# fujii-team/Henbun

Measured on AMD Instinct MI355X. Metric: elbo_samples_per_sec, higher is better.
Workload: dtype f32; 1 GPU; cfg2 SVGP ELBO step: 1-D UnitRBF, N=1e6, M=512 inducing, minibatch 8192 per GPU, diag Normal q(u), diagonal residual, Adam lr 1e-3; global_batch=8192, per_gpu_batch=8192, parallelism=dp1, N=1000000, M=512, dp_exchange=none, dp_ranks=1, contraction=native, tri_pack=False

## Files before the change

henbun_amd/csrc/elementwise.hip:

```cpp
#include "common.cuh"
#include "rng_pairs.cuh"
#include "side_jobs.cuh"
#include <string.h>
#include "../../include/henbun_hip.h"

struct EwArgs {
  int ndim;
  int nin, nout;
  int op;
  long n;
  int shape[HB_MAX_DIMS];
  long istride[4][HB_MAX_DIMS];
  const void* in[4];
  void* out[3];
  double p[4];
};

#include "ew_apply.cuh"

template <typename T>
__global__ void __launch_bounds__(256) ew_kernel(EwArgs A) {
  const long stride = (long)gridDim.x * blockDim.x;
  for (long i = (long)blockIdx.x * blockDim.x + threadIdx.x; i < A.n; i += stride) {
    long off[4] = {0, 0, 0, 0};
// ... 618 lines not shown
                                                                     const long* __restrict__ perm, long n, long nsrc,
                                                                     int* __restrict__ err) {
  gather_draw_body<T>(g, state, nlanes, lo, range, idx_out, perm, n, nsrc, err, G, (long)blockIdx.x);
}
template <typename T>
static int gather_rows_multi_draw(int narr, const T* const* srcs, const long* rows, T* const* dsts, long nsrc,
                                  uint64_t* state, long nlanes, long lo, long hi, long* idx_out, const long* perm,
                                  long n, int* err, hipStream_t stream, bool defer = false) {
  HB_REQUIRE(narr >= 1 && narr <= HB_GATHER_MAX, "hb_gather_rows_multi_draw: %d arrays (max %d)", narr, HB_GATHER_MAX);
  HB_REQUIRE(n >= 0 && nsrc >= 0 && srcs && rows && dsts && state && idx_out, "hb_gather_rows_multi_draw: bad arguments");
  HB_REQUIRE(n <= nlanes, "hb_gather_rows_multi_draw: n=%ld exceeds the %ld RNG lanes (draw with hb_rng_randint instead)", n,
             nlanes);
  HB_REQUIRE(hi > lo, "hb_gather_rows_multi_draw: empty range [%ld,%ld)", lo, hi);
  GatherMultiArgs<T> g;
  g.narr = narr;
  g.start[0] = 0;
  long wmax = 1;
  for (int a = 0; a < HB_GATHER_MAX; ++a) {
    g.src[a] = a < narr ? srcs[a] : nullptr;
    g.dst[a] = a < narr ? dsts[a] : nullptr;
    g.row[a] = a < narr ? rows[a] : 1;
    if (a < narr) HB_REQUIRE(rows[a] >= 1 && srcs[a] && dsts[a], "hb_gather_rows_multi_draw: bad array %d", a);
    if (a < narr && rows[a] > wmax) wmax = rows[a];
    g.start[a + 1] = g.start[a] + (a < narr ? n * rows[a] : 0);
  }
  if (n == 0) return 0;
  const uint64_t range = (uint64_t)(hi - lo);
  constexpr long VEC = 16 / (long)sizeof(T);
  bool vec16 = true;
  for (int a = 0; a < narr; ++a)
    vec16 = vec16 && rows[a] % VEC == 0 && ((uintptr_t)srcs[a] % 16) == 0 && ((uintptr_t)dsts[a] % 16) == 0;
  const long wsel = vec16 ? wmax / VEC : wmax;
  const int Gsel = wsel <= 2 ? 1 : (wsel <= 8 ? 4 : (wsel <= 32 ? 16 : 64));
  if constexpr (sizeof(T) == 4) {
    if (defer) {
      HbSideJob j;
      j.kind = HB_SIDE_GATHER_DRAW;
      j.gather.G = vec16 ? -Gsel : Gsel;
      j.nblocks = hb_cdiv(n * Gsel, 256);
      if (j.nblocks <= 1024) {
        memcpy(&j.gather.g, &g, sizeof(g));
        j.gather.state = state; j.gather.nlanes = nlanes; j.gather.lo = lo; j.gather.range = range;
        j.gather.idx_out = idx_out; j.gather.perm = perm; j.gather.n = n; j.gather.nsrc = nsrc; j.gather.err = err;
        return hb_side_push(j, stream);
      }
    }
  }
#define HB_GDRAW(G_)                                                                                                   \
  hipLaunchKernelGGL((gather_rows_multi_draw_kernel<T, G_>), dim3((unsigned)hb_cdiv(n * (G_ < 0 ? -(G_) : (G_)), 256)), dim3(256), 0, \
                     stream, g, state, nlanes, lo, range, idx_out, perm, n, nsrc, err)
  if (vec16) {
    if (Gsel == 1)
      HB_GDRAW(-1);
    else if (Gsel == 4)
      HB_GDRAW(-4);
    else if (Gsel == 16)
      HB_GDRAW(-16);
    else
      HB_GDRAW(-64);
  } else if (Gsel == 1)
    HB_GDRAW(1);
  else if (Gsel == 4)
    HB_GDRAW(4);
  else if (Gsel == 16)
    HB_GDRAW(16);
  else
    HB_GDRAW(64);
#undef HB_GDRAW
  HB_LAUNCH_CHECK();
  return 0;
}
extern "C" int hb_gather_rows_multi_draw_f32(int narr, const float* const* srcs, const long* rows, float* const* dsts,
                                             long nsrc, uint64_t* state, long nlanes, long lo, long hi, long* idx_out,
                                             const long* perm, long n, int* err, void* stream) {
  return gather_rows_multi_draw<float>(narr, srcs, rows, dsts, nsrc, state, nlanes, lo, hi, idx_out, perm, n, err,
                                       (hipStream_t)stream);
}
extern "C" int hb_side_push_gather_draw_f32(int narr, const float* const* srcs, const long* rows, float* const* dsts, long nsrc,
                                           uint64_t* state, long nlanes, long lo, long hi, long* idx_out, const long* perm,
                                           long n, int* err, void* stream) {
  return gather_rows_multi_draw<float>(narr, srcs, rows, dsts, nsrc, state, nlanes, lo, hi, idx_out, perm, n, err,
                                       (hipStream_t)stream, true);
}
extern "C" int hb_gather_rows_multi_draw_f64(int narr, const double* const* srcs, const long* rows, double* const* dsts,
                                             long nsrc, uint64_t* state, long nlanes, long lo, long hi, long* idx_out,
                                             const long* perm, long n, int* err, void* stream) {
  return gather_rows_multi_draw<double>(narr, srcs, rows, dsts, nsrc, state, nlanes, lo, hi, idx_out, perm, n, err,
                                        (hipStream_t)stream);
}

#define HB_GLL_BLOCK_ELEMS 1024
template <typename T>
__global__ void __launch_bounds__(256) gauss_ll_kernel(const T* __restrict__ x, const T* __restrict__ f,
                                                       const T* __restrict__ scale, const T* __restrict__ var,
                                                       long n, T* __restrict__ dmu, T* __restrict__ partial,
                                                       T* __restrict__ fbar, T post) {
  __shared__ T smem[16];
  const T s = scale ? scale[0] : T(1), v = var[0];
  const T iv = T(1) / v, lc = T(-0.91893853320467274178) - T(0.5) * hb_log(v);
  T all = T(0), asc = T(0), avr = T(0);
  const long base = (long)blockIdx.x * HB_GLL_BLOCK_ELEMS;
#pragma unroll
  for (int q = 0; q < HB_GLL_BLOCK_ELEMS / 256; ++q) {
    const long j = base + q * 256 + threadIdx.x;
    const long jc = j < n ? j : n - 1;
    const T xv = x[jc], fv = f[jc];
    const T dlt = xv - fv * s;
    const T g = dlt * iv;
    if (j < n) {
      dmu[j] = g;
      if (fbar) fbar[j] = s * (post * g);
      all += lc - T(0.5) * dlt * g;
      asc += g * fv;
      avr += T(-0.5) * iv + T(0.5) * g * g;
    }
  }
  all = block_sum(all, smem);
  asc = block_sum(asc, smem);
  avr = block_sum(avr, smem);
  if (threadIdx.x == 0) {
    partial[blockIdx.x] = all;
    partial[gridDim.x + blockIdx.x] = asc;
    partial[2 * gridDim.x + blockIdx.x] = avr;
  }
}
template <typename T>
__global__ void __launch_bounds__(256) gauss_ll_finish_kernel(const T* __restrict__ partial, int nb, T* __restrict__ ll,
                                                              T* __restrict__ dscale, T* __restrict__ dvar) {
  __shared__ T smem[16];
  T a0 = T(0), a1 = T(0), a2 = T(0);
  for (int i = threadIdx.x; i < nb; i += 256) {
    a0 += partial[i];
    a1 += partial[nb + i];
    a2 += partial[2 * nb + i];
  }
  a0 = block_sum(a0, smem);
  a1 = block_sum(a1, smem);
  a2 = block_sum(a2, smem);
  if (threadIdx.x == 0) {
    ll[0] = a0;
    dscale[0] = a1;
    dvar[0] = a2;
  }
}
#define HB_GLL_SINGLE_N 16384
template <typename T>
__global__ void __launch_bounds__(1024) gauss_ll_single_kernel(const T* __restrict__ x, const T* __restrict__ f,
                                                               const T* __restrict__ scale, const T* __restrict__ var,
                                                               long n, T* __restrict__ dmu, T* __restrict__ ll,
                                                               T* __restrict__ dscale, T* __restrict__ dvar,
                                                               T* __restrict__ fbar, T post) {
  __shared__ T smem[16];
  static_assert(HB_GLL_SINGLE_N == 16 * 1024, "hb_gauss_ll_single_body: 16 elements per thread of a 1024-thread workgroup");
  hb_gauss_ll_single_body<T>(x, f, scale, var, n, dmu, ll, dscale, dvar, smem, fbar, post);
}

template <typename T>
static int gauss_ll(const T* x, const T* f, const T* scale, const T* var, long n, T* ll, T* dmu, T* dscale, T* dvar,
                    T* ws, long ws_elems, hipStream_t stream, double post = 0.0, T* fbar = nullptr) {
  HB_REQUIRE(n >= 0 && x && f && var && ll && dmu && dscale && dvar && ws, "hb_gauss_ll: bad arguments");
  const int nb = n > 0 ? hb_cdiv(n, HB_GLL_BLOCK_ELEMS) : 0;
  HB_REQUIRE(ws_elems >= 3L * (nb > 0 ? nb : 1), "hb_gauss_ll: workspace of 3*ceil(n/%d) elements required",
             HB_GLL_BLOCK_ELEMS);
  if (hb_chain_recording()) {
    if (n > 0 && n <= HB_CHAIN_GLL_MAX_N) {
      HbChainJob j;
// ... 132 lines not shown
```

henbun_amd/csrc/linalg.hip:

```cpp
#include "common.cuh"
#include "sgp_strip.cuh"
#include "side_jobs.cuh"
#include "gemm_tile.cuh"
#include "chain.cuh"
#include "../../include/henbun_hip.h"

template <typename T>
struct MmArgs {
  const T* A;
  const T* B;
  T* C;
  long M, N, K, lda, ldb, ldc, sA, sB, sC, batch;
  T alpha, beta;
  const T* bias;
  long sBias;
  int act, flags, S, tile;
  int to_ws;
  int bfast;
  T* ws;
  T* colsum;
  T* colsum_ws;
};

template <typename T>
// ... 471 lines not shown
        dm[k] = k < d ? (Xb[(long)(row0 + r) * d + k] * il[k] - xj[k] * il[k]) : 0.f;
        r2 += dm[k] * dm[k];
      }
      const float km = hb_exp(-0.5f * r2), kb = gval[e];
      const float em = kb * km, gm = (kb + kb) * km;
#pragma unroll
      for (int k = 0; k < HB_MMG_MAXD; ++k) {
        if (k < d) {
          float ga = (-dm[k] * gm) * il[k], la = (dm[k] * dm[k] * em) * il[k];
#pragma unroll
          for (int off = 16; off > 0; off >>= 1) {
            ga += __shfl_xor(ga, off, 32);
            la += __shfl_xor(la, off, 32);
          }
          if (c == 0) {
            __hip_atomic_store(pt + r * 2 * d + k, ga, __ATOMIC_RELAXED, __HIP_MEMORY_SCOPE_AGENT);
            __hip_atomic_store(pt + r * 2 * d + d + k, la, __ATOMIC_RELAXED, __HIP_MEMORY_SCOPE_AGENT);
          }
        }
      }
    }
    asm volatile("s_waitcnt vmcnt(0)" ::: "memory");
    __shared__ unsigned s_lastg;
    __syncthreads();
    if (tid == 0) {
      const unsigned old = __hip_atomic_fetch_add(gv.counters + b * tiles_m + ti, 1u, __ATOMIC_RELAXED, __HIP_MEMORY_SCOPE_AGENT);
      s_lastg = old == (unsigned)tiles_n - 1u ? 1u : 0u;
    }
    __syncthreads();
    if (s_lastg) {
      const float* p0 = gv.part + (((long)b * tiles_m + ti) * tiles_n) * 32 * 2 * d;
      for (int idx = tid; idx < 32 * 2 * d; idx += 256) {
        float sum = 0.f;
        for (int t = 0; t < tiles_n; ++t) sum += __hip_atomic_load(const_cast<float*>(p0) + (long)t * 32 * 2 * d + idx, __ATOMIC_RELAXED, __HIP_MEMORY_SCOPE_AGENT);
        const int r = idx / (2 * d), q = idx - r * 2 * d;
        if (q < d)
          gv.Xbar[((long)b * M + row0 + r) * d + q] = sum;
        else
          gv.ell_partial[((long)b * M + row0 + r) * d + q - d] = sum;
      }
      if (tid == 0) __hip_atomic_store(gv.counters + b * tiles_m + ti, 0u, __ATOMIC_RELAXED, __HIP_MEMORY_SCOPE_AGENT);
    }
  }
  if (!SYM && (a.flags & HB_MM_SYMLOW_OUT) && ti != tj) {
#pragma unroll
    for (int e = 0; e < 4; ++e) {
      const int idx = tid + 256 * e, r = idx >> 5, c = idx & 31;
      Cb[(long)(col0 + r) * a.ldc + row0 + c] = 0.5f * a.alpha * ((red[0][c][r] + red[1][c][r]) + (red[2][c][r] + red[3][c][r]));
    }
  }
  if (SYM && ti != tj) {
#pragma unroll
    for (int e = 0; e < 4; ++e) {
      const int idx = tid + 256 * e, r = idx >> 5, c = idx & 31;
      const float v = ((red[0][c][r] + red[1][c][r]) + (red[2][c][r] + red[3][c][r])) * a.alpha;
      const float vm = ((red[4][r][c] + red[5][r][c]) + (red[6][r][c] + red[7][r][c])) * a.alpha;
      Cb[(long)(col0 + r) * a.ldc + row0 + c] = 0.5f * (v + vm);
    }
  }
}

extern "C" int hb_matmul_wgk_shape(long M, long N, long K, long batch) {
  if (M % 32 || N % 32 || K % 128 || K < 128 || K > 4096) return 0;
  return (M / 32) * (N / 32) * batch <= 1024 && batch <= 65535 ? 1 : 0;
}
template <typename T>
static bool matmul_wgk_ok(const MmArgs<T>&, long, long, long, long, int, bool) { return false; }
template <>
bool matmul_wgk_ok<float>(const MmArgs<float>& a, long M, long N, long K, long batch, int flags, bool aligned) {
  const bool off = hb_debug_get("mm_no_wgk", 0) != 0;
  if (off || !aligned || !hb_matmul_wgk_shape(M, N, K, batch)) return false;
  if (flags & HB_MM_ACTGRAD) return false;
  return !((flags & HB_MM_SYM_OUT) && M != N);
}
template <typename T>
static int matmul_wgk_launch(const MmArgs<T>&, int, int, hipStream_t) { return -1; }
int matmul_wgk_launch_g(const MmArgs<float>& a, int transA, int transB, hipStream_t stream, const MmGramVjp& gv, bool tiles = false);
template <>
int matmul_wgk_launch<float>(const MmArgs<float>& a, int transA, int transB, hipStream_t stream) { return matmul_wgk_launch_g(a, transA, transB, stream, MmGramVjp()); }
int matmul_wgk_launch_g(const MmArgs<float>& a, int transA, int transB, hipStream_t stream, const MmGramVjp& gv, bool tiles) {
  const bool sym = (a.flags & HB_MM_SYM_OUT) != 0;
  const long nt = a.M / 32;
  const int nown = (int)(sym ? nt * (nt + 1) / 2 : (a.M / 32) * (a.N / 32));
  const HbSideJobs sj = hb_side_take();
  dim3 grid((unsigned)(nown + sj.total), (unsigned)a.batch, 1);
#define HB_WGK(TA_, TB_)                                                                                   \
  do {                                                                                                     \
    if (sym)                                                                                               \
      hipLaunchKernelGGL((matmul_wgk_kernel<TA_, TB_, true>), grid, dim3(256), 0, stream, a, nown, sj, gv);    \
    else if (tiles)                                                                                        \
      hipLaunchKernelGGL((matmul_wgk_kernel<TA_, TB_, false, true>), grid, dim3(256), 0, stream, a, nown, sj, gv); \
    else                                                                                                   \
      hipLaunchKernelGGL((matmul_wgk_kernel<TA_, TB_, false>), grid, dim3(256), 0, stream, a, nown, sj, gv);   \
  } while (0)
  if (!transA && !transB)
    HB_WGK(false, false);
  else if (!transA && transB)
    HB_WGK(false, true);
  else if (transA && !transB)
    HB_WGK(true, false);
  else
    HB_WGK(true, true);
#undef HB_WGK
  HB_LAUNCH_CHECK();
  return 0;
}

#define RS_LDS_FLOATS 18432
template <bool TB, int NT, int WC, int G, int NW>
__global__ void __launch_bounds__(64 * NW, NW == 8 ? 4 : 2) matmul_rows_kernel(MmArgs<float> a) {
  typedef float V4 __attribute__((ext_vector_type(4)));
  typedef Mma<float> MM;
  __shared__ __attribute__((aligned(16))) float Ws[RS_LDS_FLOATS];
  const int M = (int)a.M, N = (int)a.N, K = (int)a.K;
  const int lda = (int)a.lda, ldb = (int)a.ldb, ldc = (int)a.ldc;
  const int KLD = K + 4;
  const int tid = threadIdx.x, lane = tid & 63, w = __builtin_amdgcn_readfirstlane(tid >> 6), li = lane & 31, h = lane >> 5;
  constexpr int NP = 32 * NT * WC, ROWS = 32 * (NW / WC), NTHR = 64 * NW;
  const int wr = w / WC, wc = w % WC;
  {
    const int kq = K >> 2;
    if (TB) {
      for (int idx = tid; idx < NP * kq; idx += NTHR) {
        const int c = idx / kq, k4 = idx - c * kq;
        V4 v = {0.f, 0.f, 0.f, 0.f};
        if (c < N) v = *reinterpret_cast<const V4*>(a.B + (long)c * ldb + 4 * k4);
        *reinterpret_cast<V4*>(&Ws[c * KLD + 4 * k4]) = v;
      }
    } else {
      for (int idx = tid; idx < NP * kq; idx += NTHR) {
        const int k4 = idx / NP, c = idx - k4 * NP;
        V4 v = {0.f, 0.f, 0.f, 0.f};
        if (c < N) {
#pragma unroll
          for (int i = 0; i < 4; ++i) v[i] = a.B[(long)(4 * k4 + i) * ldb + c];
        }
        *reinterpret_cast<V4*>(&Ws[c * KLD + 4 * k4]) = v;
      }
    }
  }
  const int cbase = 32 * NT * wc;
  float breg[NT];
#pragma unroll
  for (int t = 0; t < NT; ++t) {
    const int c = cbase + 32 * t + li;
    breg[t] = (a.bias && !(a.flags & HB_MM_ACTGRAD) && c < N) ? a.bias[c] : 0.f;
  }
  __syncthreads();
  const int nchunk = K / (2 * G);
  const int ntile = (M + ROWS - 1) / ROWS;
  for (int tile = blockIdx.x; tile < ntile; tile += gridDim.x) {
    const int r0 = tile * ROWS + 32 * wr;
    if (r0 >= M || cbase >= N) continue;
    const int arow = r0 + li < M ? r0 + li : M - 1;
    const float* __restrict__ ap = a.A + (long)arow * lda + G * h;
    typename MM::Acc acc[NT];
#pragma unroll
    for (int t = 0; t < NT; ++t)
#pragma unroll
      for (int r = 0; r < 16; ++r) acc[t][r] = 0.f;
    auto load = [&](V4 (&f)[G / 4], int c) {
      const int cc = c < nchunk ? c : nchunk - 1;
#pragma unroll
      for (int v = 0; v < G / 4; ++v) f[v] = *reinterpret_cast<const V4*>(ap + 2 * G * cc + 4 * v);
    };
    auto compute = [&](const V4 (&f)[G / 4], int c) {
      if (c >= nchunk) return;
// ... 1422 lines not shown
  HB_STAMP(1);
  if (!factor) {
    if (live) {
      T* dst = yt ? Y : L;
      const int wrow0 = adiag ? row0 - C64_NB : row0;
#pragma unroll
      for (int sj = 0; sj < 2; ++sj)
#pragma unroll
        for (int r = 0; r < 16; ++r) dst[(wrow0 + MM::acc_row(lane, r)) * M + col0 + sj * 32 + li] = acc[sj][r];
    }
    return;
  }

  if (live) {
    int fail = 0;
    int seen[2] = {0, 0};
    HB_WSTAMP(w, lane, 0);
    c64_step<0>(acc, Cs, L8s, steps_done, w, lane, fail, seen, k);
    c64_step<1>(acc, Cs, L8s, steps_done, w, lane, fail, seen, k);
    c64_step<2>(acc, Cs, L8s, steps_done, w, lane, fail, seen, k);
    c64_step<3>(acc, Cs, L8s, steps_done, w, lane, fail, seen, k);
    if (w != 0) {
      c64_step<4>(acc, Cs, L8s, steps_done, w, lane, fail, seen, k);
      c64_step<5>(acc, Cs, L8s, steps_done, w, lane, fail, seen, k);
      c64_step<6>(acc, Cs, L8s, steps_done, w, lane, fail, seen, k);
      c64_step<7>(acc, Cs, L8s, steps_done, w, lane, fail, seen, k);
    }
    if (w < 2) {
      if (fail != 0) fail = c64_locate_failure(Cs, w, lane);
      if (lane == 0) wave_fail[w] = fail;
    }
  }
  __syncthreads();
  HB_STAMP(2);
  if (s == 0 && tid == 0) {
    const int fail = wave_fail[0] != 0 ? wave_fail[0] : wave_fail[1];
    const int bad = fail != 0 ? k * C64_NB + fail : 0;
    if (k == 0)
      *info = bad;
    else if (bad != 0 && *info == 0)
      *info = bad;
  }
  constexpr int VPR = C64_NB / 4;
#pragma unroll 1
  for (int g = 0; g < 4; ++g) {
    bool glive, gy;
    int grt;
    describe(g, glive, gy, grt);
    if (!glive || (g < 2 && s != 0)) continue;
    for (int idx = tid; idx < 32 * VPR; idx += 256) {
      const int pr = idx / VPR, c = (idx % VPR) * 4;
      VT v = *reinterpret_cast<const VT*>(&Cs[g * 32 + pr][c]);
      if (g < 2) {
        const int dpr = g * 32 + pr;
#pragma unroll
        for (int e = 0; e < 4; ++e)
          if (c + e > dpr) v[e] = T(0);
      }
      *reinterpret_cast<VT*>((gy ? Y : L) + (grt * 32 + pr) * M + k * C64_NB + c) = v;
    }
    if (gy) {
      for (int idx = tid; idx < 32 * C64_NB; idx += 256) {
        const int r = idx % 32, c = idx / 32;
        W[(k * C64_NB + c) * M + grt * 32 + r] = Cs[g * 32 + r][c];
      }
    }
  }
  HB_STAMP(3);
}

#include "chol_persist.cuh"
#ifdef HB_CP_STAMPS
extern unsigned long long* hb_cp_stamps_buffer;
#endif

struct CpGram {
  const float* X = nullptr;
  const float* ell = nullptr;
  long sX = 0, sEll = 0, dl = 0, d = 0;
  int kind = 0;
  float diag = 0.f;
};
__global__ void __launch_bounds__(512, 2) chol_persist_kernel(CpArgs a, HbSideJobs side) {
  if ((int)blockIdx.x >= a.total) {
    if (threadIdx.x < 256) hb_side_run(side, (int)blockIdx.x - a.total);
    return;
  }
  __shared__ __attribute__((aligned(16))) char lds[sizeof(CpLds)];
  __shared__ unsigned s_ticket;
  if (threadIdx.x == 0) s_ticket = __hip_atomic_fetch_add(&a.sync[0], 1u, __ATOMIC_RELAXED, __HIP_MEMORY_SCOPE_AGENT);
  __syncthreads();
  chol_persist_body(a, *reinterpret_cast<CpLds*>(lds), s_ticket);
}

int hb_sgp_rider_launch_with(CpArgs& a, const HbSideJobs& sj, hipStream_t stream);
int hb_sgp_rider_launch_alone(hipStream_t stream);

static int chol_persist_launch(const float* A, const CpGram& g, float* L, float* W, float* ws, float* Wf, int bf16x3, long B, long M,
                               int* info, hipStream_t stream) {
  CpArgs a;
  a.A = A, a.L = L, a.W = W, a.X = ws;
  a.gX = g.X, a.gell = g.ell, a.gsX = g.sX, a.gsEll = g.sEll, a.gdl = g.dl, a.gd = g.d, a.gkind = g.kind, a.gdiag = g.diag;
  a.Wf = Wf, a.bf16x3 = bf16x3;
  a.sync = reinterpret_cast<unsigned*>(ws + B * M * M);
  a.info = info;
  a.M = (int)M, a.B = (int)B, a.nb = (int)(M / CP_NB);
  a.total = (int)cp_total(B, a.nb, 1);
  a.early = (hb_debug_get("chol_chunk_stores_late", 0) ? 16 : 0) | (hb_debug_get("chol_pair_prev", 0) ? 32 : 0), a.nside = 0, a.arrive = a.total, a.poll_naps = 1;
#ifdef HB_CP_STAMPS
  a.stamps = hb_cp_stamps_buffer;
#else
  a.stamps = nullptr;
#endif
  const HbSideJobs sj = hb_side_take();
  const int rr = hb_sgp_rider_launch_with(a, sj, stream);
  if (rr != 0) return rr < 0 ? rr : 0;
  hipLaunchKernelGGL(chol_persist_kernel, dim3((unsigned)(a.total + sj.total)), dim3(512), 0, stream, a, sj);
  HB_LAUNCH_CHECK();
  return hb_sgp_rider_launch_alone(stream);
}
static inline bool chol_persist_shape(long B, long M, size_t elem) {
  return elem == 4 && M >= CP_NB && M % CP_NB == 0 && M <= 8192 && B >= 1 && B * (M / CP_NB) * (M / CP_NB) <= 65536;
}
extern "C" long hb_cholesky_frag_elems(long B, long M, int bf16x3) { return hb_wfrag_layout(B, M, bf16x3 != 0).total; }
extern "C" int hb_cholesky_persistent_shape(long B, long M, int elem_bytes) {
  return chol_persist_shape(B, M, (size_t)elem_bytes) && hb_debug_get("chol_persist", 1) != 0 ? 1 : 0;
}
extern "C" int hb_gram_cholesky_inverse_f32(int kind, const float* X, long sX, const float* ell, long sEll, long dl, long d,
                                            double diag_add, float* L, float* W, long B, long M, int* info, float* ws,
                                            float* Wfrag, int frag_bf16x3, void* stream) {
  HB_REQUIRE(kind >= HB_KERN_RBF && kind < HB_KERN_SQDIST, "hb_gram_cholesky_inverse: unknown kernel kind %d", kind);
  HB_REQUIRE(X && ell && L && W && info && ws, "hb_gram_cholesky_inverse: NULL pointer");
  HB_REQUIRE(B >= 1 && d >= 1 && (dl == 1 || dl == d), "hb_gram_cholesky_inverse: bad extents");
  HB_REQUIRE(sEll == 0 || sEll == dl, "hb_gram_cholesky_inverse: lengthscale batch stride must be 0 or dl");
  HB_REQUIRE(hb_cholesky_persistent_shape(B, M, 4), "hb_gram_cholesky_inverse: fp32 with M %% 64 == 0 only (M = %ld, B = %ld)", M, B);
  HB_REQUIRE(((uintptr_t)L % 16 == 0) && ((uintptr_t)W % 16 == 0) && ((uintptr_t)ws % 16 == 0) && (!Wfrag || (uintptr_t)Wfrag % 16 == 0),
             "hb_gram_cholesky_inverse: outputs and workspace must be 16-byte aligned");
  HB_REQUIRE(!frag_bf16x3 || Wfrag, "hb_gram_cholesky_inverse: bf16x3 images need Wfrag");
  CpGram g;
  g.X = X, g.ell = ell, g.sX = sX, g.sEll = sEll, g.dl = dl, g.d = d, g.kind = kind, g.diag = (float)diag_add;
  return chol_persist_launch(nullptr, g, L, W, ws, Wfrag, frag_bf16x3, B, M, info, (hipStream_t)stream);
}
extern "C" long hb_cholesky_inverse_ws_elems(long B, long M, int elem_bytes) {
  if (B <= 0 || M <= 0) return 1;
  return B * M * M + (chol_persist_shape(B, M, (size_t)elem_bytes) ? cp_sync_words(B, M) : 0);
}

template <typename T>
static int cholesky_launch(const T* A, T* L, T* W, T* ws, T* Wf, int bf16x3, long B, long M, int* info, hipStream_t stream) {
  HB_REQUIRE(!Wf || (W && M % 32 == 0), "hb_cholesky_inverse: the fragment-major copies need W and M %% 32 == 0");
  HB_REQUIRE(!bf16x3 || (Wf && sizeof(T) == 4), "hb_cholesky_inverse: bf16x3 images need Wfrag and fp32");
  HB_REQUIRE(B >= 0 && M >= 0, "hb_cholesky: negative extent");
  HB_REQUIRE(A && L && info, "hb_cholesky: NULL pointer");
  HB_REQUIRE(!W || ws, "hb_cholesky_inverse: workspace of B*M*M elements required");
  HB_REQUIRE(B <= 65535, "hb_cholesky: batch too large");
  HB_REQUIRE(M * M < 2147483647L, "hb_cholesky: matrix too large for 32-bit indexing");
  if (B == 0) return 0;
  if (M == 0) {
    HB_HIP(hb_zero_async(info, sizeof(int) * B, stream));
    return 0;
  }
  HB_REQUIRE((const void*)A != (const void*)L && (const void*)A != (const void*)W && (const void*)L != (const void*)W,
             "hb_cholesky: A, L (and W) must not alias");
  const int inv = W != nullptr;
  const int nblk = hb_cdiv(M, CR_B);
  const bool fast = ((uintptr_t)L % 16 == 0) && ((uintptr_t)A % 16 == 0) && ((uintptr_t)ws % 16 == 0) && M % CR_B == 0;
  const bool no64 = hb_debug_get("chol_no64", 0) != 0;
  if (sizeof(T) == 4 && fast && inv && chol_persist_shape(B, M, sizeof(T)) && hb_debug_get("chol_persist", 1) != 0) {
    return chol_persist_launch((const float*)A, CpGram(), (float*)L, (float*)W, (float*)ws, (float*)Wf, bf16x3, B, M, info, stream);
  } else if (sizeof(T) == 4 && fast && M % C64_NB == 0 && !no64) {
    const int nrt = (int)(M / 32);
    HbSideJobs noside = {};
    for (int k = 0; k < nrt / 2; ++k) {
      const int nown = chol64_grid(nrt, k, inv);
      const HbSideJobs sj = k == 0 ? hb_side_take() : noside;
      dim3 grid((unsigned)(nown + (k == 0 ? sj.total : 0)), (unsigned)B);
      hipLaunchKernelGGL(chol_rl64_kernel, grid, dim3(256), 0, stream, (const float*)A, (float*)L,
                         inv ? (float*)ws : (float*)nullptr, (float*)W, (int)M, k, info, nown, sj);
      HB_LAUNCH_CHECK();
    }
  } else {
    for (int k = 0; k < nblk; ++k) {
      dim3 grid((unsigned)chol_rl_grid(nblk, k, inv), (unsigned)B);
      if (fast)
        hipLaunchKernelGGL((chol_rl_kernel<T, true>), grid, dim3(256), 0, stream, A, L, inv ? ws : (T*)nullptr, W, (int)M, k,
                           info);
      else
        hipLaunchKernelGGL((chol_rl_kernel<T, false>), grid, dim3(256), 0, stream, A, L, inv ? ws : (T*)nullptr, W, (int)M,
                           k, info);
      HB_LAUNCH_CHECK();
    }
  }
  hipLaunchKernelGGL(tril_inplace_kernel<T>, dim3(hb_stream_grid(B * M * M, 256)), dim3(256), 0, stream, L, W, Wf, bf16x3, B, M);
  HB_LAUNCH_CHECK();
  return 0;
}

extern "C" int hb_cholesky_f32(const float* A, float* L, long B, long M, int* info, void* stream) {
  return cholesky_launch<float>(A, L, nullptr, nullptr, nullptr, 0, B, M, info, (hipStream_t)stream);
}
extern "C" int hb_cholesky_f64(const double* A, double* L, long B, long M, int* info, void* stream) {
  return cholesky_launch<double>(A, L, nullptr, nullptr, nullptr, 0, B, M, info, (hipStream_t)stream);
}
extern "C" int hb_cholesky_inverse_f32(const float* A, float* L, float* W, long B, long M, int* info, float* ws,
                                       float* Wfrag, int frag_bf16x3, void* stream) {
  HB_REQUIRE(W, "hb_cholesky_inverse: NULL pointer");
  return cholesky_launch<float>(A, L, W, ws, Wfrag, frag_bf16x3, B, M, info, (hipStream_t)stream);
}
extern "C" int hb_cholesky_inverse_f64(const double* A, double* L, double* W, long B, long M, int* info, double* ws,
                                       double* Wfrag, int frag_bf16x3, void* stream) {
  HB_REQUIRE(W, "hb_cholesky_inverse: NULL pointer");
  return cholesky_launch<double>(A, L, W, ws, Wfrag, frag_bf16x3, B, M, info, (hipStream_t)stream);
}

template <typename T>
__global__ void __launch_bounds__(64) trinv_diag_kernel(const T* __restrict__ L, T* __restrict__ W, long M) {
  __shared__ __attribute__((aligned(16))) T LsT[CH_NB][CH_LD];
  __shared__ __attribute__((aligned(16))) T invd[CH_NB];
  const long b = blockIdx.y;
  L += b * M * M;
  W += b * M * M;
  const long i0 = (long)blockIdx.x * CH_NB;
  const int nb = (int)((M - i0) < CH_NB ? (M - i0) : CH_NB);
  const int lane = threadIdx.x;
  for (int idx = lane; idx < CH_NB * CH_NB; idx += 64) {
    const int i = idx / CH_NB, j = idx % CH_NB;
    const bool ok = (i < nb) & (j < nb) & (j <= i);
    const T v = L[(i0 + (i < nb ? i : 0)) * M + i0 + (j < nb ? j : 0)];
    const T val = ok ? v : (i == j ? T(1) : T(0));
    LsT[j][i] = val;
    if (i == j) invd[i] = T(1) / val;
  }
  __syncthreads();
  const int c = lane & 31;
  T t[CH_NB];
#pragma unroll
  for (int i = 0; i < CH_NB; ++i) t[i] = (i == c) ? T(1) : T(0);
  trsolve_row32<T>(t, LsT, invd);
  if (lane < nb) {
#pragma unroll
    for (int i = 0; i < CH_NB; ++i)
      if (i < nb) W[(i0 + i) * M + i0 + lane] = t[i];
  }
}

template <typename T, int PHASE, bool FAST>
__global__ void __launch_bounds__(256) trinv_level_kernel(const T* __restrict__ L, T* __restrict__ W,
                                                          T* __restrict__ Tm, long Ml, long sl) {
  typedef TileGemm<T, 64, 64, 16, 2, 2> G;
  __shared__ __attribute__((aligned(16))) T lds[G::LDS_ELEMS];
  const long b = blockIdx.z;
  L += b * Ml * Ml;
  W += b * Ml * Ml;
  Tm += b * Ml * Ml;
  const int M = (int)Ml, s = (int)sl;
  const int pair = blockIdx.y;
  const int c0 = 2 * pair * s, r0 = c0 + s;
  const int tps = (s + 63) / 64;
// ... 139 lines not shown
```

henbun_amd/csrc/runtime.hip:

```cpp
#include "common.cuh"
#include "side_jobs.cuh"
#include "../../include/henbun_hip.h"
#include <stdarg.h>
#include <stdio.h>
#include <string.h>

static thread_local char g_err[512] = "";

void hb_set_error(const char* fmt, ...) {
  va_list ap;
  va_start(ap, fmt);
  vsnprintf(g_err, sizeof(g_err), fmt, ap);
  va_end(ap);
}

extern "C" const char* hb_last_error_string(void) { return g_err; }

#include <mutex>
namespace {
struct HbDebugEntry { char key[40]; long value; };
HbDebugEntry g_dbg[32];
int g_ndbg = 0;
std::mutex g_dbg_mu;
}
long hb_debug_get(const char* key, long dflt) {
  std::lock_guard<std::mutex> lk(g_dbg_mu);
  for (int i = 0; i < g_ndbg; ++i)
    if (strcmp(g_dbg[i].key, key) == 0) return g_dbg[i].value;
  return dflt;
}
extern "C" int hb_debug_set(const char* key, long value) {
  HB_REQUIRE(key && key[0] && strlen(key) < sizeof(g_dbg[0].key), "hb_debug_set: bad key");
  std::lock_guard<std::mutex> lk(g_dbg_mu);
  for (int i = 0; i < g_ndbg; ++i)
    if (strcmp(g_dbg[i].key, key) == 0) {
      g_dbg[i].value = value;
      return 0;
    }
  HB_REQUIRE(g_ndbg < 32, "hb_debug_set: table full");
  strcpy(g_dbg[g_ndbg].key, key);
  g_dbg[g_ndbg++].value = value;
  return 0;
}
extern "C" int hb_debug_clear(void) {
  std::lock_guard<std::mutex> lk(g_dbg_mu);
  g_ndbg = 0;
  return 0;
}
extern "C" int hb_version(void) { return HB_ABI_VERSION; }

extern "C" int hb_device_info(char* buf, int buflen, int* cu_count) {
  int dev = 0;
  HB_HIP(hipGetDevice(&dev));
  hipDeviceProp_t prop;
  HB_HIP(hipGetDeviceProperties(&prop, dev));
  if (buf && buflen > 0) snprintf(buf, buflen, "%s (%s)", prop.name, prop.gcnArchName);
  if (cu_count) *cu_count = prop.multiProcessorCount;
  return 0;
}

extern "C" int hb_graph_begin_capture(void* stream) {
  HB_HIP(hipStreamBeginCapture((hipStream_t)stream, hipStreamCaptureModeThreadLocal));
  return 0;
}

extern "C" int hb_graph_end_capture(void* stream, void** exec_out) {
  HB_REQUIRE(exec_out != nullptr, "hb_graph_end_capture: exec_out is NULL");
  hipGraph_t graph = nullptr;
  HB_HIP(hipStreamEndCapture((hipStream_t)stream, &graph));
  hipGraphExec_t exec = nullptr;
  hipError_t e = hipGraphInstantiate(&exec, graph, nullptr, nullptr, 0);
  hipGraphDestroy(graph);
  if (e != hipSuccess) {
    hb_set_error("hipGraphInstantiate: %s", hipGetErrorString(e));
    return (int)e;
  }
  *exec_out = (void*)exec;
  return 0;
}

extern "C" int hb_graph_launch(void* exec, void* stream) {
  HB_REQUIRE(exec != nullptr, "hb_graph_launch: exec is NULL");
  HB_HIP(hipGraphLaunch((hipGraphExec_t)exec, (hipStream_t)stream));
  return 0;
}

extern "C" int hb_graph_destroy(void* exec) {
  if (exec) HB_HIP(hipGraphExecDestroy((hipGraphExec_t)exec));
  return 0;
}

static thread_local HbSideJobs hb_side_list = {};

__global__ void __launch_bounds__(256) hb_side_jobs_kernel(HbSideJobs J) { hb_side_run(J, (int)blockIdx.x); }

static int hb_side_launch(const HbSideJobs& J, hipStream_t stream) {
  if (J.n == 0 || J.total == 0) return 0;
  hipLaunchKernelGGL(hb_side_jobs_kernel, dim3((unsigned)J.total), dim3(256), 0, stream, J);
  HB_LAUNCH_CHECK();
  return 0;
}

HbSideJobs hb_side_take() {
  HbSideJobs J = hb_side_list;
  hb_side_list.n = 0;
  hb_side_list.total = 0;
  return J;
}

int hb_side_push(const HbSideJob& job, hipStream_t stream) {
  if (hb_side_list.n == HB_SIDE_MAX) {
    const HbSideJobs J = hb_side_take();
    const int rc = hb_side_launch(J, stream);
    if (rc) return rc;
  }
  hb_side_list.job[hb_side_list.n++] = job;
  hb_side_list.total += job.nblocks;
  return 0;
}

extern "C" int hb_side_pending(void) { return hb_side_list.n; }
extern "C" int hb_side_discard(void) {
  const int n = hb_side_list.n;
  hb_side_list.n = 0;
  hb_side_list.total = 0;
  return n;
}
extern "C" int hb_side_flush(void* stream) {
  const HbSideJobs J = hb_side_take();
  return hb_side_launch(J, (hipStream_t)stream);
}
```

henbun_amd/csrc/sgp.hip:

```cpp
#include "common.cuh"
#include "sgp_strip.cuh"
#include "chain.cuh"
#include "chol_persist.cuh"
#include <type_traits>
#include "gemm_tile.cuh"
#include "rng_pairs.cuh"
#include "../../include/henbun_hip.h"

#define SGP_BM 64
#define SGP_BN 128

extern "C" int hb_matmul_f32(const float*, const float*, float*, long, long, long, long, long, long, long, long, long,
                             long, int, int, double, double, const float*, long, int, int, float*, long, void*);
extern "C" int hb_matmul_f64(const double*, const double*, double*, long, long, long, long, long, long, long, long,
                             long, long, int, int, double, double, const double*, long, int, int, double*, long,
                             void*);

template <typename T>
struct SgpArgs {
  const T* x;
  long sx;
  const T* z;
  const T* ell;
  long dl;
// ... 1146 lines not shown
          *reinterpret_cast<V4*>(&slot[(v * 64 + lane) * 4]) = q;
        }
        asm volatile("" ::: "memory");
        __hip_atomic_store(st, 2 * p - 1, __ATOMIC_RELAXED, __HIP_MEMORY_SCOPE_WORKGROUP);
        asm volatile("" ::: "memory");
      }
    }
  }

  sgp_2t_epilogue<true>(a, lds_raw, csq, cu, e, bx, col0, n, means);
  cp_arrive(ca, *reinterpret_cast<unsigned*>(ctl + 3));
}

template <int D>
__global__ void __launch_bounds__(512, 4) chol_sgp_fwd_kernel(CpArgs ca, HbSideJobs side, SgpArgs<float> a) {
  __shared__ __attribute__((aligned(16))) char lds[SGP_E_LDS_BYTES];
  __shared__ unsigned s_ticket;
  if (threadIdx.x == 0) s_ticket = __hip_atomic_fetch_add(&ca.sync[0], 1u, __ATOMIC_RELAXED, __HIP_MEMORY_SCOPE_AGENT);
  __syncthreads();
  const unsigned t = s_ticket;
  if (t < (unsigned)ca.total) {
    chol_persist_body(ca, *reinterpret_cast<CpLds*>(lds), t);
    return;
  }
  if (t < (unsigned)(ca.total + ca.nside)) {
    if (threadIdx.x >= 256) return;
    hb_side_run(side, (int)t - ca.total);
    __syncthreads();
    if (threadIdx.x == 0) __hip_atomic_fetch_add(&ca.sync[3], 1u, __ATOMIC_RELEASE, __HIP_MEMORY_SCOPE_AGENT);
    return;
  }
  if (ca.early & 2) {
    cp_arrive(ca, s_ticket);
    return;
  }
  sgp_early_body<D>(a, ca, lds, (int)t - ca.total - ca.nside);
}


static inline int sgp_grid_y(long E, long n, int nRB) {
  const long paired = (long)hb_cdiv(n, SGP_BN) * ((nRB + 1) / 2) * E;
  return (paired < 384 && nRB > 1) ? nRB : (nRB + 1) / 2;
}

struct SgpWs {
  long ellpart;
  long shared;
  long mm_elems;
  long strip_elems;
  long slabs;
  long slab_cap;
  long total;
};
static inline SgpWs sgp_ws(long E, long n, long M, long d, long P) {
  SgpWs w;
  const long gy = (M + SGP_BM - 1) / SGP_BM;
  const long fwd_part = 5 * E * gy * n, nS = hb_cdiv(n, SGP_SN);
  w.ellpart = E * n, w.shared = w.ellpart + E * M * d;
  w.mm_elems = 32 * E * M * M, w.strip_elems = nS * (2 * d + P) * M * E;
  const long padded = ((w.strip_elems + 63) / 64) * 64;
  w.slabs = w.shared + padded;
  w.slab_cap = E * M > 0 ? (w.mm_elems - padded) / (E * M * M) : 0;
  w.total = w.shared + (w.mm_elems > fwd_part ? w.mm_elems : fwd_part);
  return w;
}
extern "C" long hb_sgp_ws_elems(long E, long n, long M, long d, long P) { return sgp_ws(E, n, M, d, P).total; }

enum { SGP_CALL_FWD, SGP_CALL_A, SGP_CALL_BWD };
#define SGP_FK_DMAX 2
#define SGP_FK_MAX_STRIPS 512
enum { SGP_K_TILED, SGP_K_STRIP, SGP_K_STRIP2, SGP_K_STRIP2T, SGP_K_STRIP16, SGP_K_STRIP3 };
struct SgpForm {
  bool path;
  int kernel;
  bool partials;
  int part_rows;
  bool fin;
  long head_units;
  bool record;
  bool rider;
  bool bwd_strip;
  bool bwd_phi;
  bool fwd_kbar;
  SgpWs ws;
};
static SgpForm sgp_form(int call, int elem_bytes, long E, long n, long M, long d, long P, int prec, bool has_wfrag, bool w_aligned,
                        bool has_ws, bool draw, long rng_lanes, bool want_xbar) {
  const bool no_strip = hb_debug_get("sgp_no_strip", 0) != 0;
  const bool force_strip = hb_debug_get("sgp_force_strip", 0) != 0;
  const bool old_crossover = hb_debug_get("sgp_tiled_crossover", 0) != 0;
  const bool form2 = hb_debug_get("sgp_strip_form2", 0) != 0;
  const bool no_fused_finish = hb_debug_get("sgp_no_fused_finish", 0) != 0;
  const bool form16 = hb_debug_get("sgp_form16", 0) != 0;
  const bool early = hb_debug_get("sgp_early", 1) != 0;
  const bool phi_direct = hb_debug_get("sgp_phi_direct", 1) != 0;
  const bool fwd_kbar = hb_debug_get("sgp_fwd_kbar", 1) != 0;
  SgpForm f;
  f.ws = sgp_ws(E, n, M, d, P);
  const bool fp32 = elem_bytes == 4, bf16x3 = prec == HB_PREC_BF16X3;
  const long nS = hb_cdiv(n, SGP_SN);
  const long tiled_wgs = E * hb_cdiv(n, SGP_BN) * ((hb_cdiv(M, SGP_BM) + 1) / 2);
  const bool strip_M = M >= 32 && M <= SGP_SM_MAX && M % 32 == 0;
  f.path = !no_strip && strip_M && d >= 1 && d <= SGP_DREG && P <= 4 && n > 0 && E >= 1 &&
           (bf16x3 || (old_crossover ? tiled_wgs < 1024 && E * nS <= 4096 : E * nS <= (1L << 22) && nS * (2 * d + P) <= 31 * M));
  const bool plain_strip = !no_strip && strip_M && d <= SGP_DREG && w_aligned && (tiled_wgs < 1024 || force_strip);
  f.partials = call != SGP_CALL_A && M > 0 && P <= 4 && has_ws;
  const bool strip = fp32 && (call == SGP_CALL_A ? plain_strip || bf16x3 : f.partials && ((has_wfrag && f.path) || plain_strip));
  const bool form3 = (!f.partials || P <= 1) && !form2;
  f.kernel = !strip ? SGP_K_TILED : bf16x3 ? SGP_K_STRIP3 : !has_wfrag ? SGP_K_STRIP : !form3 ? SGP_K_STRIP2
             : (form16 && M >= 384) ? SGP_K_STRIP16 : SGP_K_STRIP2T;
  f.part_rows = strip ? 1 : sgp_grid_y(E, n, hb_cdiv(M, SGP_BM));
  f.fin = call == SGP_CALL_FWD && strip && has_wfrag && !bf16x3 && f.path && !no_fused_finish && !form2 && P <= 1 && n % 2 == 0 &&
          (!draw || rng_lanes >= (E * n + 1) / 2);
  f.head_units = f.fin && P == 1 ? E * nS : 0;
  f.record = f.fin && d <= SGP_E_DMAX;
  f.rider = f.record && early && M % CP_NB == 0 && hb_cholesky_persistent_shape(E, M, 4);
  f.bwd_strip = fp32 && has_wfrag && !want_xbar && f.path && f.ws.strip_elems <= f.ws.mm_elems;
  f.bwd_phi = !bf16x3 && f.path && phi_direct;
  f.fwd_kbar = f.head_units > 0 && f.bwd_phi && f.bwd_strip && d <= SGP_FK_DMAX && E * nS <= SGP_FK_MAX_STRIPS && fwd_kbar;
  return f;
}
static inline SgpForm sgp_form_query(long E, long n, long M, long d, long P, int prec, bool has_wfrag, bool draw, long rng_lanes) {
  return sgp_form(SGP_CALL_FWD, 4, E, n, M, d, P, prec, has_wfrag, true, true, draw, rng_lanes, false);
}

struct SgpRider {
  bool armed = false, valid = false;
  SgpArgs<float> a;
  SgpForm form;
  long E = 0;
};
static thread_local SgpRider g_rider;
static int sgp_A_strip_launch(SgpArgs<float> a, long E, int kernel, hipStream_t stream);
struct SgpFwdKbar {
  const float* WTf;
  float* part;
  float* Abf;
};
static int sgp_fwd_kbar_launch(SgpArgs<float> a, SgpFwdKbar k, long E, hipStream_t stream);

extern "C" int hb_sgp_rider_supported(long E, long n, long M, long d, long P, int prec, int has_wfrag, int draw, long rng_lanes) {
  return sgp_form_query(E, n, M, d, P, prec, has_wfrag != 0, draw != 0, rng_lanes).rider ? 1 : 0;
}
extern "C" int hb_sgp_rider_begin(void) {
  HB_REQUIRE(!g_rider.valid, "hb_sgp_rider_begin: a recorded forward is still pending (hb_sgp_rider_flush)");
  g_rider.armed = true;
  return 0;
}
extern "C" int hb_sgp_rider_pending(void) { return g_rider.valid ? 1 : 0; }
int hb_sgp_rider_launch_alone(hipStream_t stream) {
  g_rider.armed = false;
  if (!g_rider.valid) return 0;
  g_rider.valid = false;
  return sgp_A_strip_launch(g_rider.a, g_rider.E, g_rider.form.kernel, stream);
}
extern "C" int hb_sgp_rider_flush(void* stream) { return hb_sgp_rider_launch_alone((hipStream_t)stream); }

int hb_sgp_rider_launch_with(CpArgs& ca, const HbSideJobs& sj, hipStream_t stream) {
  if (!g_rider.valid) return 0;
  const SgpArgs<float>& a = g_rider.a;
  const long E = g_rider.E, nS = hb_cdiv(a.n, SGP_SN);
  static int cus = 0;
  if (cus == 0 && (hb_device_info(nullptr, 0, &cus) || cus <= 0)) cus = 256;
  const bool ok = g_rider.form.rider && a.Wf == ca.Wf && !ca.bf16x3 && E == ca.B && a.M == ca.M &&
                  (long)ca.total + sj.total + E * nS <= 2L * cus;
  if (!ok) return 0;
  ca.early = 1 | ((int)(hb_debug_get("sgp_early_diag", 0) & 3) << 1), ca.nside = sj.total, ca.arrive = ca.total + (int)(E * nS);
  g_rider.valid = false, g_rider.armed = false;
  ca.poll_naps = (int)hb_debug_get("sgp_early_poll_naps", 1);
  long nunits = E * nS;
  if (hb_debug_get("sgp_early_diag", 0) == 4) nunits = 0, ca.arrive = ca.total;
  const dim3 grid((unsigned)(ca.total + sj.total + nunits));
  if (a.d == 1)
    hipLaunchKernelGGL((chol_sgp_fwd_kernel<1>), grid, dim3(512), 0, stream, ca, sj, a);
  else
    hipLaunchKernelGGL((chol_sgp_fwd_kernel<2>), grid, dim3(512), 0, stream, ca, sj, a);
  HB_LAUNCH_CHECK();
  return 1;
}

#define SGP_S3LD (SGP_SM_MAX + 8)
template <int D>
__global__ void __launch_bounds__(SGP_STRIP_THREADS) sgp_A_strip3_kernel(SgpArgs<float> a) {
  typedef float V4 __attribute__((ext_vector_type(4)));
  typedef __bf16 B8 __attribute__((ext_vector_type(8)));
  typedef Mma<float> MM;
  __shared__ __attribute__((aligned(16))) __bf16 K3[3][SGP_SN][SGP_S3LD];
  __shared__ __attribute__((aligned(16))) float zs[SGP_SM_MAX * D];
  __shared__ float us[4][SGP_SM_MAX];
  __shared__ __attribute__((aligned(16))) float Tw[SGP_STRIP_THREADS / 64][32][SGP_TLD];
  long e;
  int bx;
  sgp_block(a.efast, e, bx);
  const float* __restrict__ x = a.x + e * a.sx;
  const float* __restrict__ z = a.z + e * a.M * D;
  const float* __restrict__ ell = a.ell + e * a.dl;
  const __bf16* __restrict__ W3 = reinterpret_cast<const __bf16*>(a.W3) + e * a.M * a.M;
  float* __restrict__ A = a.A ? a.A + e * a.M * a.n : nullptr;
  const int M = (int)a.M, n = (int)a.n;
  const int col0 = bx * SGP_SN;
  const int tid = threadIdx.x, lane = tid & 63, w = __builtin_amdgcn_readfirstlane(tid >> 6), li = lane & 31, h = lane >> 5;

  {
    const int c = tid & 31, kq = tid >> 5;
    constexpr int NTH = SGP_STRIP_THREADS;
    SgpStripColumn<D> col;
    SgpStageZ<D, NTH> zst;
    SgpStageU<NTH> ust;
    const int npu = a.part ? ((int)a.P < 4 ? (int)a.P : 4) : 0;
    col.load(x, ell, a.dl, col0, n, tid);
    zst.request(z, M, tid);
    ust.request(a.u + e * a.P * a.M, npu, M, tid);
    zst.store(zs, M, tid);
    ust.store(us, npu, M, tid);
    __syncthreads();
#pragma unroll 2
    for (int k8 = kq * 8; k8 < M; k8 += NTH / 4) {
      B8 p0, p1, p2;
#pragma unroll
      for (int q = 0; q < 8; ++q) {
// ... 253 lines not shown

template <typename T>
struct SgpHead {
  const T* y = nullptr;
  const T* scale = nullptr;
  const T* var = nullptr;
  double post = 0.0;
  T* dmu = nullptr;
  T* fbar = nullptr;
  T* part = nullptr;
  long units = 0;
};
extern "C" long hb_sgp_head_units(long E, long n, long M, long d, long P, int prec, int has_wfrag, int draw, long rng_lanes) {
  return sgp_form_query(E, n, M, d, P, prec, has_wfrag != 0, draw != 0, rng_lanes).head_units;
}

template <typename T>
static SgpArgs<T> sgp_args(const T* x, long sx, const T* z, const T* ell, long dl, const T* W, const T* Wf, int prec, const T* u,
                           T* A, T* A_frag, T* part, long E, long n, long M, long d, long P) {
  const HbWfragLayout lay = hb_wfrag_layout(E, M, prec == HB_PREC_BF16X3);
  SgpArgs<T> a;
  a.x = x; a.sx = sx; a.z = z; a.ell = ell; a.dl = dl; a.W = W; a.Wf = Wf; a.u = u; a.A = A;
  a.n = n; a.M = M; a.d = d; a.P = P;
  a.W3 = Wf && prec == HB_PREC_BF16X3 ? lay.w3(Wf) : nullptr;
  a.plane3 = Wf ? lay.plane : 0;
  a.Af = A_frag;
  a.part = part;
  return a;
}

template <typename T>
static int sgp_fwd(int kind, int mode, const T* x, long sx, const T* z, const T* ell, long dl, const T* W, const T* Wf,
                   int prec, const T* u, const T* eps_in, uint64_t* rng, long rng_lanes, T* eps_out, T* A, T* A_frag, T* f,
                   T* v, long E, long n, long M, long d, long P, T* ws, hipStream_t stream, const SgpHead<T>* head = nullptr,
                   const SgpFwdKbar* fk = nullptr) {
  const bool diag = mode == HB_SGP_DIAGONAL, draw = diag && !eps_in;
  const T* fin_eps_in = diag ? eps_in : nullptr;
  uint64_t* fin_rng = draw ? rng : nullptr;
  T* fin_eps_out = diag ? eps_out : nullptr;
  const SgpForm form = sgp_form(SGP_CALL_FWD, (int)sizeof(T), E, n, M, d, P, prec, Wf != nullptr, (uintptr_t)W % 16 == 0, ws != nullptr,
                                draw, rng_lanes, false);
  HB_REQUIRE(!A_frag || (sizeof(T) == 4 && Wf && ws && form.path),
             "hb_sgp_fwd: a fragment-major A needs the column-strip form (fp32, Wfrag, hb_sgp_strip_path)");
  if (hb_chain_recording()) {
    const int crc = hb_chain_flush(stream);
    if (crc) return crc;
  }
  HB_REQUIRE(prec == HB_PREC_NATIVE || prec == HB_PREC_BF16X3, "hb_sgp_fwd: unknown precision %d", prec);
  HB_REQUIRE(prec == HB_PREC_NATIVE || (sizeof(T) == 4 && Wf && M % 32 == 0 && M <= SGP_SM_MAX && d <= SGP_DREG && P <= 4 && ws),
             "hb_sgp_fwd: bf16x3 needs fp32, the bf16 images in Wfrag, M %% 32 == 0, M <= %d, d <= %d, P <= 4", SGP_SM_MAX, SGP_DREG);
  HB_REQUIRE(kind == HB_KERN_RBF, "hb_sgp_fwd: only the UnitRBF kernel is fused (kind=%d)", kind);
  HB_REQUIRE(mode == HB_SGP_NEGLECTED || mode == HB_SGP_DIAGONAL, "hb_sgp_fwd: unknown mode %d", mode);
  HB_REQUIRE(E >= 0 && n >= 0 && M >= 0 && d >= 1 && P >= 0, "hb_sgp_fwd: bad extents");
  HB_REQUIRE(dl == 1 || dl == d, "hb_sgp_fwd: lengthscales must have 1 or d entries");
  HB_REQUIRE(x && z && ell && W && u && (A || A_frag) && f && v, "hb_sgp_fwd: NULL pointer");
  HB_REQUIRE(E <= 65535, "hb_sgp_fwd: too many experts");
  HB_REQUIRE(M * n < 2147483647L && M * M < 2147483647L && n * d < 2147483647L, "hb_sgp_fwd: matrix too large for 32-bit indexing");
  if (E * n == 0) return 0;
  if (draw) HB_REQUIRE(rng && rng_lanes > 0 && eps_out, "hb_sgp_fwd: need eps_in, or rng and eps_out");
  HB_REQUIRE(!head || (M > 0 && P == 1 && ws && Wf), "hb_sgp_fwd_gauss: needs Wfrag, a workspace and P == 1");
  if (form.partials) {
    SgpArgs<T> a = sgp_args<T>(x, sx, z, ell, dl, W, Wf, prec, u, A, A_frag, ws + form.ws.shared, E, n, M, d, P);
    const int gyp = form.part_rows;
    int rc;
    a.fin = 0;
    if (form.kernel != SGP_K_TILED) {
      if (form.fin) {
        a.fin = 1, a.fin_diag = diag, a.fin_eps_in = fin_eps_in, a.fin_rng = fin_rng, a.fin_lanes = rng_lanes;
        a.fin_eps_out = fin_eps_out, a.fin_f = f, a.fin_v = v;
        if (head) {
          HB_REQUIRE(form.head_units > 0 && head->units == form.head_units, "hb_sgp_fwd_gauss: units must be hb_sgp_head_units(...)");
          a.head = 1;
          a.hy = head->y, a.hscale = head->scale, a.hvar = head->var;
          a.hdmu = head->dmu, a.hfbar = head->fbar, a.hpost = (T)head->post;
          a.hpart = head->part, a.hunits = head->units;
        }
      }
      HB_REQUIRE(!head || a.fin, "hb_sgp_fwd_gauss: this call cannot carry the head (hb_sgp_head_units(...) == 0)");
      if constexpr (std::is_same<T, float>::value) {
        if (fk) {
          HB_REQUIRE(form.fwd_kbar && a.head && a.hfbar && A_frag, "hb_sgp_fwd_gauss_kbar: not served here (hb_sgp_fwd_kbar_supported), or fbar / A_frag missing");
          HB_REQUIRE(!A, "hb_sgp_fwd_gauss_kbar: A is exchanged fragment-major only (pass A = NULL)");
          HB_REQUIRE(!g_rider.armed, "hb_sgp_fwd_gauss_kbar after hb_sgp_rider_begin: the fused call does not ride");
          return sgp_fwd_kbar_launch(a, *fk, E, stream);
        }
        if (g_rider.armed) {
          HB_REQUIRE(form.record, "hb_sgp_fwd after hb_sgp_rider_begin: this call cannot ride (hb_sgp_rider_supported)");
          sgp_grid(hb_cdiv(a.n, SGP_SN), 1, E, a.efast);
          g_rider.a = a, g_rider.form = form, g_rider.E = E, g_rider.valid = true, g_rider.armed = false;
          return 0;
        }
      }
      rc = sgp_A_strip_launch(a, E, form.kernel, stream);
      if (rc) return rc;
      if (a.fin) return 0;
    } else {
      dim3 grid = sgp_grid(hb_cdiv(n, SGP_BN), gyp, E, a.efast);
      rc = sgp_A_launch<T>(a, grid, stream);
    }
    if (rc) return rc;
    const long total = E * n;
    if (hb_chain_recording() && total <= HB_CHAIN_FINISH_MAX_N) {
      HbChainJob j;
      j.kind = HB_CHAIN_SGP_FINISH;
      j.is64 = sizeof(T) == 8;
      j.p[0] = a.part, j.p[1] = fin_eps_in, j.p[2] = fin_rng, j.p[3] = fin_eps_out, j.p[4] = f, j.p[5] = v;
      j.l[0] = gyp, j.l[1] = rng_lanes, j.l[2] = total, j.l[3] = n, j.l[4] = P, j.l[5] = diag;
      const long tb = total * (long)sizeof(T);
      j.span(0, tb * gyp * 5, HB_CHAIN_READ), j.span(1, tb, HB_CHAIN_READ), j.span(2, 2 * rng_lanes * (long)sizeof(uint64_t), HB_CHAIN_RW);
      j.span(3, tb, HB_CHAIN_WRITE), j.span(4, tb * P, HB_CHAIN_WRITE), j.span(5, tb, HB_CHAIN_WRITE);
      return hb_chain_push(j, stream);
    }
    const int fgrid = draw ? hb_cdiv(rng_lanes, 256) : hb_stream_grid((total + 1) / 2, 256);
    hipLaunchKernelGGL(sgp_finish_part_kernel<T>, dim3(fgrid), dim3(256), 0, stream, a.part, gyp, fin_eps_in, fin_rng, rng_lanes,
                       fin_eps_out, f, v, total, n, P, mode);
    HB_LAUNCH_CHECK();
    return 0;
  }
  const T* eps = eps_in;
  if (mode == HB_SGP_DIAGONAL) {
    if (draw) {
      hipLaunchKernelGGL(sgp_rng_fill_kernel<T>, dim3(hb_cdiv(rng_lanes, 256)), dim3(256), 0, stream, rng, rng_lanes,
                         eps_out, E * n);
      HB_LAUNCH_CHECK();
      eps = eps_out;
    } else if (eps_out && eps_out != eps_in) {
      HB_HIP(hb_copy_async(eps_out, eps_in, sizeof(T) * E * n, stream));
    }
  }
  if (M > 0) {
    SgpArgs<T> a = sgp_args<T>(x, sx, z, ell, dl, W, nullptr, HB_PREC_NATIVE, u, A, nullptr, nullptr, E, n, M, d, P);
    dim3 grid = sgp_grid(hb_cdiv(n, SGP_BN), form.part_rows, E, a.efast);
    int rc = sgp_A_launch<T>(a, grid, stream);
    if (rc) return rc;
  }
  hipLaunchKernelGGL(sgp_finish_kernel<T>, dim3(hb_cdiv(n, 32), (unsigned)E), dim3(256), 0, stream, A, u, eps, f, v, n,
                     M, P, mode);
  HB_LAUNCH_CHECK();
  return 0;
}

template <typename T>
static int sgp_A_only(int kind, const T* x, long sx, const T* z, const T* ell, long dl, const T* W, const T* Wf, int prec,
                      T* A, long E, long n, long M, long d, hipStream_t stream) {
  HB_REQUIRE(prec == HB_PREC_NATIVE || prec == HB_PREC_BF16X3, "hb_sgp_A: unknown precision %d", prec);
  HB_REQUIRE(prec == HB_PREC_NATIVE || (sizeof(T) == 4 && Wf && M % 32 == 0 && M <= SGP_SM_MAX && d <= SGP_DREG),
             "hb_sgp_A: bf16x3 needs fp32, the bf16 images in Wfrag, M %% 32 == 0, M <= %d, d <= %d", SGP_SM_MAX, SGP_DREG);
  HB_REQUIRE(kind == HB_KERN_RBF, "hb_sgp_A: only the UnitRBF kernel is fused (kind=%d)", kind);
  HB_REQUIRE(E >= 0 && n >= 0 && M >= 0 && d >= 1, "hb_sgp_A: bad extents");
  HB_REQUIRE(dl == 1 || dl == d, "hb_sgp_A: lengthscales must have 1 or d entries");
  HB_REQUIRE(x && z && ell && W && A, "hb_sgp_A: NULL pointer");
  HB_REQUIRE(E <= 65535, "hb_sgp_A: too many experts");
  HB_REQUIRE(M * n < 2147483647L && M * M < 2147483647L && n * d < 2147483647L, "hb_sgp_A: matrix too large");
  if (E * n * M == 0) return 0;
  SgpArgs<T> a = sgp_args<T>(x, sx, z, ell, dl, W, Wf, prec, nullptr, A, nullptr, nullptr, E, n, M, d, 0);
  const SgpForm form = sgp_form(SGP_CALL_A, (int)sizeof(T), E, n, M, d, 0, prec, Wf != nullptr, (uintptr_t)W % 16 == 0, false, false, 0, false);
  if (form.kernel != SGP_K_TILED) return sgp_A_strip_launch(a, E, form.kernel, stream);
  dim3 grid = sgp_grid(hb_cdiv(n, SGP_BN), form.part_rows, E, a.efast);
  return sgp_A_launch<T>(a, grid, stream);
}
extern "C" int hb_sgp_A_f32(int kind, const float* x, long sx, const float* z, const float* ell, long dl,
                            const float* W, const float* Wfrag, int prec, float* A, long E, long n, long M, long d,
                            void* stream) {
  return sgp_A_only<float>(kind, x, sx, z, ell, dl, W, Wfrag, prec, A, E, n, M, d, (hipStream_t)stream);
}
extern "C" int hb_sgp_A_f64(int kind, const double* x, long sx, const double* z, const double* ell, long dl,
                            const double* W, const double* Wfrag, int prec, double* A, long E, long n, long M, long d,
// ... 485 lines not shown
        compute(fb2, ts + 1);
        __builtin_amdgcn_sched_barrier(0);
      }
    }
  } else {
    const __bf16* __restrict__ W3 = reinterpret_cast<const __bf16*>(a.WT3) + e * a.M * a.M;
    struct Frag {
      B8 f[3][2];
    };
    auto load = [&](Frag& fr, int ts) {
      const int tc = ts < nts ? ts : nts - 1;
      const __bf16* p = W3 + ((long)(tile_of(tc) * nT + chunk_of(tc)) << 10) + 8 * lane;
#pragma unroll
      for (int t = 0; t < 3; ++t)
#pragma unroll
        for (int q = 0; q < 2; ++q) fr.f[t][q] = *reinterpret_cast<const B8*>(p + (long)t * a.plane3 + 512 * q);
    };
    auto compute = [&](const Frag& fr, int ts) {
      if (ts >= nts) return;
      const int Q = chunk_of(ts);
#pragma unroll
      for (int q = 0; q < 2; ++q) {
        B8 b[3];
#pragma unroll
        for (int t = 0; t < 3; ++t) b[t] = *reinterpret_cast<const B8*>(&K3[t][li][32 * Q + 16 * q + 8 * h]);
        acc = __builtin_amdgcn_mfma_f32_32x32x16_bf16(b[0], fr.f[2][q], acc, 0, 0, 0);
        acc = __builtin_amdgcn_mfma_f32_32x32x16_bf16(b[2], fr.f[0][q], acc, 0, 0, 0);
        acc = __builtin_amdgcn_mfma_f32_32x32x16_bf16(b[1], fr.f[1][q], acc, 0, 0, 0);
        acc = __builtin_amdgcn_mfma_f32_32x32x16_bf16(b[0], fr.f[1][q], acc, 0, 0, 0);
        acc = __builtin_amdgcn_mfma_f32_32x32x16_bf16(b[1], fr.f[0][q], acc, 0, 0, 0);
        acc = __builtin_amdgcn_mfma_f32_32x32x16_bf16(b[0], fr.f[0][q], acc, 0, 0, 0);
      }
      if (ts == d0 - 1 || ts == nts - 1) retire(tile_of(ts));
    };
    if (nts > 0) {
      Frag fa, fb2;
      load(fa, 0);
#pragma nounroll
      for (int ts = 0; ts < nts; ts += 2) {
        load(fb2, ts + 1);
        __builtin_amdgcn_sched_barrier(0);
        compute(fa, ts);
        __builtin_amdgcn_sched_barrier(0);
        load(fa, ts + 2);
        __builtin_amdgcn_sched_barrier(0);
        compute(fb2, ts + 1);
        __builtin_amdgcn_sched_barrier(0);
      }
    }
  }
  HB_KSTAMP(2);
  __syncthreads();
  float* red = lred;
#pragma unroll
  for (int dd = 0; dd < D; ++dd) {
    const float t = wave_sum(lwave[dd]);
    if (lane == 0) red[w * D + dd] = t;
  }
  __syncthreads();
#pragma unroll
  for (int dd = 0; dd < D; ++dd)
    if (tid == dd) {
      float t = 0.f;
      for (int ww = 0; ww < SGP_STRIP_THREADS / 64; ++ww) t += red[ww * D + dd];
      part[(long)(D + dd) * M] = t * col.sc[dd] * float(1.0 / (SGP_EXP2_SCALE * SGP_EXP2_SCALE * SGP_EXP2_SCALE));
    }
  HB_KSTAMP(3);
}

#ifndef HB_FSTAMP
#define HB_FSTAMP(i)
#endif
template <int D>
__global__ void __launch_bounds__(SGP_STRIP_THREADS, 4) sgp_fwd_kbar_strip_kernel(SgpArgs<float> a, SgpFwdKbar k) {
  typedef float V4 __attribute__((ext_vector_type(4)));
  typedef Mma<float> MM;
  constexpr int KS_FLOATS = SGP_SN * SGP_SLD, RED_FLOATS = 2 * SGP_SN * SGP_RED_LD;
  __shared__ __attribute__((aligned(16))) float lds_raw[KS_FLOATS > RED_FLOATS ? KS_FLOATS : RED_FLOATS];
  __shared__ __attribute__((aligned(16))) float zs[SGP_SM_MAX * D];
  __shared__ __attribute__((aligned(16))) float xss[SGP_SN * D];
  __shared__ __attribute__((aligned(16))) float cjs[SGP_SN];
  __shared__ __attribute__((aligned(16))) float fbs[1][SGP_SN];
  __shared__ float lred[(SGP_STRIP_THREADS / 64) * D];
  float (*Ks)[SGP_SLD] = reinterpret_cast<float (*)[SGP_SLD]>(lds_raw);
  long e;
  int bx;
  sgp_block(a.efast, e, bx);
  const float* __restrict__ x = a.x + e * a.sx;
  const float* __restrict__ z = a.z + e * a.M * D;
  const float* __restrict__ ell = a.ell + e * a.dl;
  const float* __restrict__ Wf = a.Wf + e * a.M * a.M;
  const int M = (int)a.M, n = (int)a.n;
  const int col0 = bx * SGP_SN;
  const int tid = threadIdx.x, lane = tid & 63, w = __builtin_amdgcn_readfirstlane(tid >> 6), li = lane & 31, h = lane >> 5;
  const int nT = M / 32;
  const int t1 = nT - 1 - w, t0 = w;
  const int d0 = w < t1 ? w + 1 : 0;
  const int d1 = w <= t1 ? t1 + 1 : 0;
  const int nts = d0 + d1;
  const bool means = true;
  HB_FSTAMP(0);
  float u0 = 0.f, u1 = 0.f;
  {
    const float* up = a.u + e * a.P * a.M;
    if (d0) u0 = up[32 * t0 + li];
    if (d1) u1 = up[32 * t1 + li];
  }
  SgpStripColumn<D> col;
  SgpStageZ<D, SGP_STRIP_THREADS> zst;
  col.load(x, ell, a.dl, col0, n, tid);
  zst.request(z, M, tid);
  zst.store(zs, M, tid);
  if (tid < SGP_SN) {
#pragma unroll
    for (int dd = 0; dd < D; ++dd) xss[tid * D + dd] = col.xs[dd];
  }
  __syncthreads();
  sgp_strip_fill<D, SGP_STRIP_THREADS>(Ks, zs, col, M, tid);
  __syncthreads();
  HB_FSTAMP(1);

  float csq[16], cu[16];
#pragma unroll
  for (int r = 0; r < 16; ++r) csq[r] = 0.f, cu[r] = 0.f;
  typename MM::Acc acc;
#pragma unroll
  for (int r = 0; r < 16; ++r) acc[r] = 0.f;
  const int nS = (n + SGP_SN - 1) / SGP_SN;
  float keep0[16], keep1[16];
#pragma unroll
  for (int i = 0; i < 16; ++i) keep0[i] = 0.f, keep1[i] = 0.f;

  {
    auto retire_fwd = [&](int tile, float um, float (&keep)[16]) {
      typedef float V2 __attribute__((ext_vector_type(2)));
      const V2 um2 = {um, um};
#pragma unroll
      for (int r = 0; r < 16; r += 2) {
        const V2 av = {acc[r], acc[r + 1]};
        const V2 q2 = __builtin_elementwise_fma(av, av, V2{csq[r], csq[r + 1]});
        const V2 m2 = __builtin_elementwise_fma(um2, av, V2{cu[r], cu[r + 1]});
        csq[r] = q2[0], csq[r + 1] = q2[1];
        cu[r] = m2[0], cu[r + 1] = m2[1];
      }
      sgp_acc_t_settle(acc);
      sgp_acc_t_rows(acc, keep);
      sgp_store_frag_rows(a.Af, keep, e, nT, nS, tile, bx, col0, n, lane);
#pragma unroll
      for (int r = 0; r < 16; ++r) acc[r] = 0.f;
    };
    auto load = [&](V4 (&f)[4], int ts) {
      const int tc = ts < nts ? ts : nts - 1;
      const int tile = tc < d0 ? t0 : t1, Q = tc < d0 ? tc : tc - d0;
      const float* p = Wf + ((long)(tile * nT + Q) << 10) + 4 * lane;
#pragma unroll
      for (int v = 0; v < 4; ++v) f[v] = *reinterpret_cast<const V4*>(p + 256 * v);
    };
    auto compute = [&](const V4 (&f)[4], int ts) {
      if (ts >= nts) return;
      const int Q = ts < d0 ? ts : ts - d0;
      V4 bv[4];
#pragma unroll
      for (int v = 0; v < 4; ++v) bv[v] = *reinterpret_cast<const V4*>(&Ks[li][32 * Q + 16 * h + 4 * v]);
#pragma unroll
      for (int v = 0; v < 4; ++v)
#pragma unroll
        for (int s = 0; s < 4; ++s) acc = MM::mma(bv[v][s], f[v][s], acc);
      if (ts == d0 - 1) retire_fwd(t0, u0, keep0);
    };
    if (nts > 0) {
      V4 fa[4], fb[4];
      load(fa, 0);
#pragma nounroll
      for (int ts = 0; ts < nts; ts += 2) {
        load(fb, ts + 1);
        __builtin_amdgcn_sched_barrier(0);
        compute(fa, ts);
        __builtin_amdgcn_sched_barrier(0);
        load(fa, ts + 2);
        __builtin_amdgcn_sched_barrier(0);
        compute(fb, ts + 1);
        __builtin_amdgcn_sched_barrier(0);
      }
      retire_fwd(t1, u1, keep1);
    }
  }
  HB_FSTAMP(2);

  const int ta = nT - 1 - w, tb = w;
  const int kd0 = ta > tb ? w + 1 : 0;
  const int kd1 = tb <= ta ? nT - w : 0;
  const int knts = kd0 + kd1;
  auto tile_of = [&](int ts) { return ts < kd0 ? ta : tb; };
  auto chunk_of = [&](int ts) { return ts < kd0 ? ta + ts : tb + (ts - kd0); };
  const float* __restrict__ WTf = k.WTf + e * a.M * a.M;
  auto kload = [&](V4 (&f)[4], int ts) {
    const int tc = ts < knts ? ts : knts - 1;
    const float* p = WTf + ((long)(tile_of(tc) * nT + chunk_of(tc)) << 10) + 4 * lane;
#pragma unroll
    for (int v = 0; v < 4; ++v) f[v] = *reinterpret_cast<const V4*>(p + 256 * v);
  };
  V4 fa[4], fb2[4];
  if (knts > 0) kload(fa, 0);
  {
    const float* ell2 = ell;
    asm volatile("" : "+s"(ell2));
    col.scale(ell2, a.dl);
  }

  sgp_2t_epilogue<false>(a, lds_raw, csq, cu, e, bx, col0, n, means, cjs, &fbs[0][0]);
  HB_FSTAMP(3);
  __syncthreads();

  const int nq = 2 * D + 1;
  float* __restrict__ part = k.part + ((e * nS + bx) * (long)nq) * M;
  auto abar_tile = [&](const float (&rows)[16], int t, float um) {
    const int kk = 32 * t + li;
    float usum = 0.f;
    float* blk = k.Abf + ((((long)e * nT + t) * nS + bx) << 10) + 4 * lane;
#pragma unroll
    for (int v = 0; v < 4; ++v) {
      const V4 ab4 = sgp_abar_group1(&rows[4 * v], um, cjs, fbs[0], h, v, usum);
#pragma unroll
      for (int s2 = 0; s2 < 4; ++s2) Ks[16 * h + 4 * v + s2][kk] = ab4[s2];
      *reinterpret_cast<V4*>(blk + 256 * v) = ab4;
    }
    const float tsum = usum + __shfl_xor(usum, 32);
    if (h == 0) part[(long)(2 * D) * M + kk] = tsum;
  };
  if (d0) abar_tile(keep0, t0, u0);
  if (d1) abar_tile(keep1, t1, u1);
  __syncthreads();
  HB_FSTAMP(4);

#pragma unroll
  for (int r = 0; r < 16; ++r) acc[r] = 0.f;
  float lwave[D];
#pragma unroll
  for (int dd = 0; dd < D; ++dd) lwave[dd] = 0.f;
  auto retire = [&](int tile) {
    sgp_acc_t_settle(acc);
    float kb[16];
    sgp_acc_t_rows(acc, kb);
    if (col0 + SGP_SN > n) {
#pragma unroll
      for (int i = 0; i < 16; ++i)
        if (col0 + 16 * h + i >= n) kb[i] = 0.f;
    }
    const int row = 32 * tile + li;
    float zr[D], zacc[D], lacc[D];
#pragma unroll
    for (int dd = 0; dd < D; ++dd) zr[dd] = zs[row * D + dd], zacc[dd] = 0.f, lacc[dd] = 0.f;
#pragma unroll
    for (int i = 0; i < 16; ++i) {
      const int c = 16 * h + i;
      float tt[D], r2 = 0.f;
#pragma unroll
      for (int dd = 0; dd < D; ++dd) {
        tt[dd] = (zr[dd] - xss[c * D + dd]) * col.sc[dd];
        r2 += tt[dd] * tt[dd];
      }
      const float gk = kb[i] * hb_exp2_neg<float>(r2);
#pragma unroll
      for (int dd = 0; dd < D; ++dd) {
        zacc[dd] -= gk * tt[dd];
        lacc[dd] += gk * tt[dd] * tt[dd];
      }
    }
#pragma unroll
    for (int dd = 0; dd < D; ++dd) {
      zacc[dd] += __shfl_xor(zacc[dd], 32);
      if (h == 0) part[(long)dd * M + row] = zacc[dd] * col.sc[dd] * float(1.0 / (SGP_EXP2_SCALE * SGP_EXP2_SCALE));
      lwave[dd] += lacc[dd];
    }
#pragma unroll
    for (int r = 0; r < 16; ++r) acc[r] = 0.f;
  };
  auto kcompute = [&](const V4 (&f)[4], int ts) {
    if (ts >= knts) return;
    const int Q = chunk_of(ts);
    V4 bv[4];
#pragma unroll
    for (int v = 0; v < 4; ++v) bv[v] = *reinterpret_cast<const V4*>(&Ks[li][32 * Q + 16 * h + 4 * v]);
#pragma unroll
    for (int v = 0; v < 4; ++v)
#pragma unroll
      for (int s2 = 0; s2 < 4; ++s2) acc = MM::mma(bv[v][s2], f[v][s2], acc);
    if (ts == kd0 - 1 || ts == knts - 1) retire(tile_of(ts));
  };
  if (knts > 0) {
#pragma nounroll
    for (int ts = 0; ts < knts; ts += 2) {
      kload(fb2, ts + 1);
      __builtin_amdgcn_sched_barrier(0);
      kcompute(fa, ts);
      __builtin_amdgcn_sched_barrier(0);
      kload(fa, ts + 2);
      __builtin_amdgcn_sched_barrier(0);
      kcompute(fb2, ts + 1);
      __builtin_amdgcn_sched_barrier(0);
    }
  }
  HB_FSTAMP(5);
  __syncthreads();
#pragma unroll
  for (int dd = 0; dd < D; ++dd) {
    const float t = wave_sum(lwave[dd]);
    if (lane == 0) lred[w * D + dd] = t;
  }
  __syncthreads();
#pragma unroll
  for (int dd = 0; dd < D; ++dd)
    if (tid == dd) {
      float t = 0.f;
      for (int ww = 0; ww < SGP_STRIP_THREADS / 64; ++ww) t += lred[ww * D + dd];
      part[(long)(D + dd) * M] = t * col.sc[dd] * float(1.0 / (SGP_EXP2_SCALE * SGP_EXP2_SCALE * SGP_EXP2_SCALE));
    }
  HB_FSTAMP(6);
}

#ifndef HB_LSTAMP
#define HB_LSTAMP(i)
#endif
template <bool BF3>
__global__ void __launch_bounds__(256) sgp_lbar_frag_kernel(const float* __restrict__ Kf, const float* __restrict__ Af,
                                                            float* __restrict__ slabs, int M, int nS, int S, long E,
                                                            int pairs, int gran) {
  typedef __bf16 B8 __attribute__((ext_vector_type(8)));
  typedef float V4 __attribute__((ext_vector_type(4)));
  typedef Mma<float> MM;
  typedef std::integral_constant<bool, true> Yes;
  typedef std::integral_constant<bool, false> No;
  __shared__ float red[4][32][33];
  const int nT = M / 32, nB = (nT + 1) / 2;
  const int U = gridDim.x, xcd = blockIdx.x & 7, kx = blockIdx.x >> 3;
  const int uq = U >> 3, ur = U & 7;
  const int unit = xcd * uq + (xcd < ur ? xcd : ur) + kx;
  const int group = unit / pairs, pair = unit - group * pairs;
  const int slab = group % S;
  const long e = group / S;
  int bi = (int)((sqrtf(8.f * (float)pair + 1.f) - 1.f) * 0.5f);
  while (bi * (bi + 1) / 2 > pair) --bi;
  while ((bi + 1) * (bi + 2) / 2 <= pair) ++bi;
  const int bj = pair - bi * (bi + 1) / 2;
  (void)nB;
  const int tid = threadIdx.x, lane = tid & 63, w = __builtin_amdgcn_readfirstlane(tid >> 6);
  const int nU = 4 * nS / gran;
  const int base = nU / S, rem = nU % S;
  const int sb = slab * base + (slab < rem ? slab : rem), se = sb + base + (slab < rem ? 1 : 0);
  const int cnt = se - sb, wq = cnt / 4, wr = cnt % 4;
  const int u0 = sb + w * wq + (w < wr ? w : wr);
  const int q0 = gran * u0, q1 = gran * (u0 + wq + (w < wr ? 1 : 0));
  const int ti0 = 2 * bi, ti1 = 2 * bi + 1 < nT ? 2 * bi + 1 : ti0, tj0 = 2 * bj, tj1 = 2 * bj + 1 < nT ? 2 * bj + 1 : tj0;
  const bool has_i1 = 2 * bi + 1 < nT, has_j1 = 2 * bj + 1 < nT;
  const bool upper01 = bi == bj;
  const long tstride = (long)nS << 10;
  const float* __restrict__ kbase = Kf + (long)e * nT * tstride + 4 * lane;
  const float* __restrict__ abase = Af + (long)e * nT * tstride + 4 * lane;
  HB_LSTAMP(0);
  typename MM::Acc acc[4];
#pragma unroll
  for (int q = 0; q < 4; ++q)
#pragma unroll
    for (int r = 0; r < 16; ++r) acc[q][r] = 0.f;
  if (!BF3) {
    struct Frag {
      V4 a0[4], a1[4], b0[4], b1[4];
    };
    const int tail = (q1 - q0) & 3, qf = q0 + tail;
    auto load_quarter = [&](Frag& f, int v, int q) {
      const int qc = q < q1 ? q : q1 - 1;
      const long off = (long)qc << 8;
// ... 905 lines not shown
```

henbun_amd/csrc/sgp_strip.cuh:

```cuda
#ifndef HB_SGP_STRIP_CUH
#define HB_SGP_STRIP_CUH
#include "common.cuh"

#define SGP_EXP2_SCALE 0.84932180028801904272
template <typename T> __device__ __forceinline__ T hb_exp2_neg(T x);
template <> __device__ __forceinline__ float hb_exp2_neg<float>(float x) { return __builtin_amdgcn_exp2f(-x); }
template <> __device__ __forceinline__ double hb_exp2_neg<double>(double x) { return exp2(-x); }

#define SGP_SN 32
#define SGP_SM_MAX 512
#define SGP_SLD (SGP_SM_MAX + 4)
#define SGP_DREG 4

template <int D>
struct SgpStripColumn {
  float sc[D], xs[D];
  __device__ __forceinline__ void scale(const float* __restrict__ ell, long dl) {
#pragma unroll
    for (int dd = 0; dd < D; ++dd) sc[dd] = float(SGP_EXP2_SCALE) / ell[dl == 1 ? 0 : dd];
  }
  __device__ __forceinline__ void load(const float* __restrict__ x, const float* __restrict__ ell, long dl, int col0, int n,
                                       int tid) {
    const int c = col0 + (tid & 31), cc = c < n ? c : n - 1;
    scale(ell, dl);
#pragma unroll
    for (int dd = 0; dd < D; ++dd) xs[dd] = x[cc * D + dd];
  }
  __device__ __forceinline__ float value(const float* zk) const {
    float r2 = 0.f;
#pragma unroll
    for (int dd = 0; dd < D; ++dd) {
      const float tt = (zk[dd] - xs[dd]) * sc[dd];
      r2 += tt * tt;
    }
    return hb_exp2_neg<float>(r2);
  }
};

template <int D, int NTH>
struct SgpStageZ {
  static constexpr int ZIT = (SGP_SM_MAX * D) / NTH;
  static_assert(ZIT >= 1, "staging loop");
  float zt[ZIT];
  __device__ __forceinline__ void request(const float* __restrict__ z, int M, int tid) {
#pragma unroll
    for (int it = 0, i = tid; it < ZIT; ++it, i += NTH) zt[it] = z[i < M * D ? i : 0];
  }
  __device__ __forceinline__ void store(float* zs, int M, int tid) const {
#pragma unroll
    for (int it = 0, i = tid; it < ZIT; ++it, i += NTH)
      if (i < M * D) zs[i] = zt[it];
  }
};
template <int NTH>
struct SgpStageU {
  static constexpr int UIT = SGP_SM_MAX / NTH;
  static_assert(UIT >= 1, "staging loop");
  float ut[4][UIT];
  __device__ __forceinline__ void request(const float* __restrict__ u_e, int np, int M, int tid) {
#pragma unroll
    for (int p = 0; p < 4; ++p)
#pragma unroll
      for (int it = 0, i = tid; it < UIT; ++it, i += NTH) ut[p][it] = p < np ? u_e[(long)p * M + (i < M ? i : 0)] : 0.f;
  }
  __device__ __forceinline__ void store(float (*us)[SGP_SM_MAX], int np, int M, int tid) const {
#pragma unroll
    for (int p = 0; p < 4; ++p)
#pragma unroll
      for (int it = 0, i = tid; it < UIT; ++it, i += NTH)
        if (p < np && i < M) us[p][i] = ut[p][it];
  }
};

template <int D, int NTH>
__device__ __forceinline__ void sgp_strip_fill(float (*Ks)[SGP_SLD], const float* zs, const SgpStripColumn<D>& col, int M, int tid) {
  typedef float V4 __attribute__((ext_vector_type(4)));
  const int c = tid & 31, kq = tid >> 5;
#pragma unroll 4
  for (int k4 = kq * 4; k4 < M; k4 += NTH / 8) {
    float zq[4 * D];
#pragma unroll
    for (int q = 0; q < 4 * D; q += 4) {
      const V4 zz = *reinterpret_cast<const V4*>(&zs[k4 * D + q]);
#pragma unroll
      for (int s = 0; s < 4; ++s) zq[q + s] = zz[s];
    }
    V4 v;
#pragma unroll
    for (int q = 0; q < 4; ++q) v[q] = col.value(&zq[q * D]);
    *reinterpret_cast<V4*>(&Ks[c][k4]) = v;
  }
}

#define SGP_TLD 36
__device__ __forceinline__ void sgp_store_frag_tile(float* __restrict__ Xf, float (*T)[SGP_TLD],
                                                    const Mma<float>::Acc& acc, long e, int nT, int nS, int tile, int strip,
                                                    int col0, int n, int lane) {
  typedef float V4 __attribute__((ext_vector_type(4)));
  const int li = lane & 31, h = lane >> 5;
#pragma unroll
  for (int r = 0; r < 16; ++r) T[Mma<float>::acc_row(lane, r)][li] = acc[r];
  float* blk = Xf + ((((long)e * nT + tile) * nS + strip) << 10) + 4 * lane;
#pragma unroll
  for (int v = 0; v < 4; ++v) {
    V4 q = *reinterpret_cast<const V4*>(&T[li][16 * h + 4 * v]);
#pragma unroll
    for (int s2 = 0; s2 < 4; ++s2)
      if (col0 + 16 * h + 4 * v + s2 >= n) q[s2] = 0.f;
    *reinterpret_cast<V4*>(blk + 256 * v) = q;
  }
}

__device__ __forceinline__ void sgp_acc_t_settle(Mma<float>::Acc& acc) {
  asm volatile("s_nop 15\n\ts_nop 3" : "+v"(acc));
}
__device__ __forceinline__ void sgp_acc_t_rows(Mma<float>::Acc& acc, float (&row16)[16]) {
  float lo[8], hi[8];
#pragma unroll
  for (int r = 0; r < 8; ++r) {
    lo[r] = acc[r], hi[r] = acc[8 + r];
    asm volatile("s_nop 1\n\tv_permlane32_swap_b32 %0, %1" : "+v"(lo[r]), "+v"(hi[r]));
  }
#pragma unroll
  for (int s = 0; s < 4; ++s) {
    row16[s] = lo[s];
    row16[4 + s] = hi[s];
    row16[8 + s] = lo[4 + s];
    row16[12 + s] = hi[4 + s];
  }
}
__device__ __forceinline__ void sgp_store_frag_rows(float* __restrict__ Xf, float (&row16)[16], long e, int nT, int nS,
                                                    int tile, int strip, int col0, int n, int lane) {
  typedef float V4 __attribute__((ext_vector_type(4)));
  const int h = lane >> 5;
  float* blk = Xf + ((((long)e * nT + tile) * nS + strip) << 10) + 4 * lane;
  if (col0 + 32 > n) {
#pragma unroll
    for (int i = 0; i < 16; ++i)
      if (col0 + 16 * h + i >= n) row16[i] = 0.f;
  }
#pragma unroll
  for (int v = 0; v < 4; ++v) {
    const V4 q = {row16[4 * v], row16[4 * v + 1], row16[4 * v + 2], row16[4 * v + 3]};
    *reinterpret_cast<V4*>(blk + 256 * v) = q;
  }
}

typedef float SgpV4 __attribute__((ext_vector_type(4)));
__device__ __forceinline__ SgpV4 sgp_abar_group1(const float* a4, float u, const float* cjs, const float* fbs, int h, int v,
                                                 float& usum) {
  const SgpV4 cj4 = *reinterpret_cast<const SgpV4*>(&cjs[16 * h + 4 * v]);
  const SgpV4 fb4 = *reinterpret_cast<const SgpV4*>(&fbs[16 * h + 4 * v]);
  SgpV4 ab4;
#pragma unroll
  for (int s2 = 0; s2 < 4; ++s2) {
    const float aval = a4[s2];
    ab4[s2] = __builtin_fmaf(u, fb4[s2], aval * cj4[s2]);
    usum = __builtin_fmaf(fb4[s2], aval, usum);
  }
  return ab4;
}

#endif
```

henbun_amd/csrc/side_jobs.cuh:

```cuda
#ifndef HB_SIDE_JOBS_CUH
#define HB_SIDE_JOBS_CUH
#include "common.cuh"
#include "rng_pairs.cuh"

#define HB_GATHER_MAX 8
template <typename T>
struct GatherMultiArgs {
  const T* src[HB_GATHER_MAX];
  T* dst[HB_GATHER_MAX];
  long row[HB_GATHER_MAX];
  long start[HB_GATHER_MAX + 1];
  int narr;
};

template <typename T>
__device__ __forceinline__ void gather_draw_body(const GatherMultiArgs<T>& g, uint64_t* __restrict__ state, long nlanes, long lo,
                                                 uint64_t range, long* __restrict__ idx_out, const long* __restrict__ perm,
                                                 long n, long nsrc, int* __restrict__ err, int Gs, long vblock) {
  const bool vec16 = Gs < 0;
  const int G = vec16 ? -Gs : Gs;
  const long t = vblock * 256 + threadIdx.x;
  const long r = t / G;
  const int sub = (int)(t % G);
  long j = 0;
// ... 32 lines not shown
    for (long c = sub; c < w; c += G) g.dst[a][r * w + c] = bad ? T(0) : g.src[a][j * w + c];
  }
}

template <typename T>
__device__ __forceinline__ void diag_fwd_body(const T* __restrict__ mu, const T* __restrict__ s, const T* __restrict__ u_in,
                                              uint64_t* rng, long rng_lanes, T* __restrict__ u_out, T* __restrict__ x,
                                              T* __restrict__ partial, T* __restrict__ kl, long n, long L, long ldm, long lds_,
                                              long vblock, long nvblocks, T* smem) {
  const bool dense = ldm == L && lds_ == L;
  auto src = [&](long i, long ld) -> long {
    if (dense) return i;
    const long r = i / L;
    return r * ld + (i - r * L);
  };
  const long t = vblock * 256 + threadIdx.x;
  const long nthreads = rng ? rng_lanes : nvblocks * 256;
  const long npairs = (n + 1) / 2;
  T acc = T(0);
  const bool active = t < nthreads && t < npairs;
  HbRng g;
  if (rng && active) g = rng_load(rng, rng_lanes, t);
  if (active) {
    for (long p = t; p < npairs; p += nthreads) {
      const long i0 = 2 * p, i1 = 2 * p + 1;
      T u0, u1 = T(0);
      if (rng) {
        T z0, z1;
        g.normal2(z0, z1);
        u0 = (T)z0;
        u1 = (T)z1;
      } else {
        u0 = u_in[i0];
        if (i1 < n) u1 = u_in[i1];
      }
      {
        const T sv = s[src(i0, lds_)];
        const T xv = mu[src(i0, ldm)] + hb_exp(sv) * u0;
        x[i0] = xv;
        if (u_out) u_out[i0] = u0;
        acc += T(2) * sv + u0 * u0 - xv * xv;
      }
      if (i1 < n) {
        const T sv = s[src(i1, lds_)];
        const T xv = mu[src(i1, ldm)] + hb_exp(sv) * u1;
        x[i1] = xv;
        if (u_out) u_out[i1] = u1;
        acc += T(2) * sv + u1 * u1 - xv * xv;
      }
    }
  }
  if (rng && active) rng_store(rng, rng_lanes, t, g);
  acc = block_sum(acc, smem);
  if (threadIdx.x == 0) {
    if (nvblocks == 1)
      kl[0] = T(-0.5) * acc;
    else
      partial[vblock] = acc;
  }
}

template <typename T>
__device__ __forceinline__ void diag_bwd_body(const T* __restrict__ s, const T* __restrict__ u, const T* __restrict__ x,
                                              const T* __restrict__ xbar, const T* __restrict__ klbar, T* __restrict__ mubar,
                                              T* __restrict__ sbar, long n, long L, long lds_, long ldo, long vblock,
                                              long nvblocks) {
  const T kb = klbar ? klbar[0] : T(0);
  const long stride = nvblocks * 256;
  const bool dense = lds_ == L && ldo == L;
  for (long i = vblock * 256 + threadIdx.x; i < n; i += stride) {
    long is = i, io = i;
    if (!dense) {
      const long r = i / L, c = i - r * L;
      is = r * lds_ + c;
      io = r * ldo + c;
    }
    const T mb = (xbar ? xbar[i] : T(0)) + kb * x[i];
    mubar[io] = mb;
    sbar[io] = mb * hb_exp(s[is]) * u[i] - kb;
  }
}

#define HB_SIDE_MAX 3
enum { HB_SIDE_GATHER_DRAW = 1, HB_SIDE_DIAG_FWD = 2, HB_SIDE_DIAG_BWD = 3 };
struct HbSideGather {
  GatherMultiArgs<float> g;
  uint64_t* state;
  long nlanes, lo;
  uint64_t range;
  long* idx_out;
  const long* perm;
  long n, nsrc;
  int* err;
  int G;
};
struct HbSideDiagFwd {
  const float *mu, *s, *u_in;
  uint64_t* rng;
  long rng_lanes;
  float *u_out, *x, *kl;
  long n, L, ldm, lds;
};
struct HbSideDiagBwd {
  const float *s, *u, *x, *xbar, *klbar;
  float *mubar, *sbar;
  long n, L, lds, ldo;
};
struct HbSideJob {
  int kind, nblocks;
  union {
    HbSideGather gather;
    HbSideDiagFwd dfwd;
    HbSideDiagBwd dbwd;
  };
};
struct HbSideJobs {
  int n, total;
  HbSideJob job[HB_SIDE_MAX];
};

__device__ __forceinline__ void hb_side_run(const HbSideJobs& J, int vb) {
  __shared__ float side_smem[16];
  if (threadIdx.x < 16) side_smem[threadIdx.x] = 0.f;
#pragma unroll
  for (int q = 0; q < HB_SIDE_MAX; ++q) {
    if (q >= J.n) return;
    const HbSideJob& j = J.job[q];
    if (vb < j.nblocks) {
      if (j.kind == HB_SIDE_GATHER_DRAW)
        gather_draw_body<float>(j.gather.g, j.gather.state, j.gather.nlanes, j.gather.lo, j.gather.range, j.gather.idx_out,
                                j.gather.perm, j.gather.n, j.gather.nsrc, j.gather.err, j.gather.G, vb);
      else if (j.kind == HB_SIDE_DIAG_FWD)
        diag_fwd_body<float>(j.dfwd.mu, j.dfwd.s, j.dfwd.u_in, j.dfwd.rng, j.dfwd.rng_lanes, j.dfwd.u_out, j.dfwd.x, nullptr,
                             j.dfwd.kl, j.dfwd.n, j.dfwd.L, j.dfwd.ldm, j.dfwd.lds, vb, 1, side_smem);
      else if (j.kind == HB_SIDE_DIAG_BWD)
        diag_bwd_body<float>(j.dbwd.s, j.dbwd.u, j.dbwd.x, j.dbwd.xbar, j.dbwd.klbar, j.dbwd.mubar, j.dbwd.sbar, j.dbwd.n,
                             j.dbwd.L, j.dbwd.lds, j.dbwd.ldo, vb, j.nblocks);
      return;
    }
    vb -= j.nblocks;
  }
}

int hb_side_push(const HbSideJob& job, hipStream_t stream);
HbSideJobs hb_side_take();

#endif
```

henbun_amd/graph.py:

```python
from __future__ import annotations

import itertools
import math
from typing import Dict, List, Optional, Sequence, Tuple

import numpy as np

from ._lib import HipBackendError as _HipBackendError
from ._lib import constants as _constants
from ._settings import settings as _settings

MATUTIL_BAND, MATUTIL_ADD_EYE, MATUTIL_PHI, MATUTIL_SYM, MATUTIL_SYMLOW = (
    _constants()["HB_MATUTIL_" + k] for k in ("BAND", "ADD_EYE", "PHI", "SYM", "SYMLOW"))

_uid = itertools.count()



class Node:
    __slots__ = ("op", "inputs", "attrs", "outputs", "id")

    def __init__(self, op, inputs, attrs, out_shapes):
        self.op = op
        self.inputs = tuple(inputs)
# ... 1704 lines not shown
    if node.attrs.get("sym"):
        oX, oL = [plan.out(t) for t in node.outputs]
        tmp = plan.scratch((B, n, d)) if (BX == 1 and B > 1) else None
        ws = plan.scratch((max(B * n * d, 1),))

        ksym = k | (H.KERN_KBAR_SYMMETRIC if tg.node.attrs.get("sym_result") else 0)

        def sym_step():
            dst = tmp if tmp is not None else oX
            H.gram_bwd_raw(ksym, X, sX, X2, sX2, ell, sEll, dl, g, dst, dst, oL, B, n, n2, d, ws)
            if tmp is not None:
                H.reduce_mid(tmp, 1, B, n * d, out=oX)

        plan.steps.append(sym_step)
        if tmp is None:
            plan.chain_kind[id(sym_step)] = "tail"
        return
    oX, oX2, oL = [plan.out(t) for t in node.outputs]
    tmpX = plan.scratch((B, n, d)) if (BX == 1 and B > 1) else None
    tmpX2 = plan.scratch((B, n2, d)) if (BX2 == 1 and B > 1) else None
    ws = plan.scratch((max(B * n * d, 1),))

    def step():
        H.gram_bwd_raw(k, X, sX, X2, sX2, ell, sEll, dl, g, tmpX if tmpX is not None else oX,
                       tmpX2 if tmpX2 is not None else oX2, oL, B, n, n2, d, ws)
        if tmpX is not None:
            H.reduce_mid(tmpX, 1, B, n * d, out=oX)
        if tmpX2 is not None:
            H.reduce_mid(tmpX2, 1, B, n2 * d, out=oX2)

    plan.steps.append(step)
    if tmpX is None and tmpX2 is None:
        plan.chain_kind[id(step)] = "tail"


defop("gram", _gram_emit, _gram_vjp)
defop("gram_grad", _gram_grad_emit, None)

SGP_MODES = {"neglected": 0, "diagonal": 1}


def sgp_samples(x, z, ell, L, u, mode="diagonal", eps=None) -> Tuple[Tensor, Tensor, Tensor, Tensor]:
    x, z, ell, L, u = (as_tensor(t) for t in (x, z, ell, L, u))
    W = stop_gradient(trinv(L))
    M, n, P = z.shape[-2], x.shape[-2], u.shape[-2]
    lead = z.shape[:-2]
    ins = [x, z, ell, L, W, u] + ([as_tensor(eps)] if eps is not None else [])
    nd = make("sgp", tuple(ins), {"mode": mode}, [lead + (P, n), lead + (M, n), lead + (n,), lead + (n,)],
              unique=(eps is None and mode == "diagonal"))
    return tuple(nd.outputs)


def _sgp_emit(plan, node):
    H = plan.H
    x, z, ell, L, W, u = (plan.buf(t) for t in node.inputs[:6])
    eps_in = plan.buf(node.inputs[6]) if len(node.inputs) > 6 else None
    outs = tuple(plan.out(t) for t in node.outputs)
    mode = SGP_MODES[node.attrs["mode"]]
    rng = plan.rng("local") if (eps_in is None and mode == 1) else None
    Wsrc = _through(node.inputs[4], ("stop_gradient",))
    wfrag, bf3 = plan._wfrag.get(Wsrc, (None, False))
    E, M, n, d, P = _sgp_extents(node)
    bf3 = bf3 and d <= 4 and P <= 4
    prec = H.PREC_BF16X3 if bf3 else H.PREC_NATIVE
    a_frag, skip_a = None, False
    if wfrag is not None and _sgp_frag_exchange(plan, node, prec):
        a_frag = plan.scratch((H.sgp_frag_elems(E, n, M, prec),))
        plan._afrag[node.outputs[1]] = (a_frag, prec)
        skip_a = node.outputs[1] not in plan.outputs
    head = None
    g = plan._sgp_head.get(node.id)
    if g is not None and wfrag is not None:
        units = H.sgp_head_units(x, z, u, prec, True, eps_in is None and mode == 1, rng)
        if units > 0:
            head = _gauss_head(plan, g, units)
    gn, why = _fwd_kbar_match(plan, node, g, head, a_frag, skip_a, prec)
    cell = plan._chol_rider.get(Wsrc) if _runtime("early_forward") else None
    if gn is not None and cell is not None:
        gn, why = None, "settings.runtime.early_forward is on: the forward is offered to the factorisation's launch, and the fused call never rides"
    if gn is not None and not H.sgp_fwd_kbar_supported(x, z, u, prec, True, eps_in is None and mode == 1, rng):
        gn, why = None, "d > 2, more than 512 strips, or switched off (hb_debug_set sgp_fwd_kbar 0)"
    if g is not None:
        plan.note(FWD_KBAR, node, gn is not None, why or "")
    if gn is not None:
        abar_frag = plan.scratch((a_frag.numel(),))
        bws = plan.scratch((H.sgp_ws_elems(E, n, M, d, P),))
        plan._fwd_kbar[gn.id] = (abar_frag, bws)
        fouts = (outs[0], outs[2], outs[3])
        step = lambda: H.sgp_fwd_gauss_kbar(x, z, ell, W, u, wfrag, a_frag, abar_frag, bws, head, eps_in=eps_in, rng=rng,
                                            mode=mode, out=fouts)
        plan.steps.append(step)
        plan.step_labels[id(step)], plan.step_nodes[id(step)] = "sgp+kbar", node
        plan.chain_kind[id(step)] = "tail"
        return
    step = lambda: H.sgp_fwd(x, z, ell, W, u, eps_in=eps_in, rng=rng, mode=mode, out=outs, wfrag=wfrag,
                             prec=prec, a_frag=a_frag, skip_a=skip_a, head=head)
    ep = "forward contraction starts inside the persistent Cholesky's launch (hb_sgp_rider_begin)"
    if cell is not None and cell["rider"] is None:
        if not H.sgp_rider_supported(x, z, u, prec, wfrag is not None, eps_in is None and mode == 1, rng):
            plan.note(ep, node, False, "needs the fused finishing pass (fp32, one latent function, d <= 2, M % 64 == 0)")
        else:
            reads = [node.inputs[0], node.inputs[1], node.inputs[2], node.inputs[5]] + list(node.inputs[6:])
            if head is not None:
                reads += [g.inputs[0], g.inputs[2]] + list(g.inputs[3:4])
            early_nodes = {id(nd) for nd in plan._emitted[:cell["epos"]]}

            def ready(t):
                src = _through(t, ("reshape", "stop_gradient")).node
                return src.op.startswith("leaf:") or id(src) in early_nodes

            if all(ready(t) for t in reads):
                cell["rider"] = step
                plan.step_labels[id(cell["step"])] = "cholesky+sgp"
                plan.step_riders[id(cell["step"])] = node
                plan.note(ep, node, True)
                return
            plan.note(ep, node, False, "an operand is produced after the factorisation has been launched")
    plan.steps.append(step)
    plan.chain_kind[id(step)] = "tail"


def _sgp_vjp(node, gs):
    gf = gs[0]
    if gf is None:
        return [None] * len(node.inputs)
    if any(g is not None for g in gs[1:3]):
        raise NotImplementedError("gradients through the A / v outputs of sgp_samples")
    x, z, ell, L, W, u = node.inputs[:6]
    f, A, v, eps = node.outputs
    n = make("sgp_grad", (x, z, ell, W, u, eps, A, v, gf), {"mode": node.attrs["mode"]},
             [L.shape, u.shape, z.shape, ell.shape, x.shape])
    Lb, ub, zb, lb, xb = n.outputs
    return [xb, zb, lb, Lb, None, ub] + [None] * (len(node.inputs) - 6)


PHI_DIRECT = "Cholesky VJP's first product folded into the sparse-GP backward (hb_sgp_bwd_phi)"
FWD_KBAR = "forward and Kbar column strips in one launch (hb_sgp_fwd_gauss_kbar)"


def _fwd_kbar_match(plan, node, g, head, a_frag, skip_a, prec):
    if g is None or head is None:
        return None, "no likelihood head rides in the forward contraction"
    if head.get("fbar") is None:
        return None, "the head does not write dobjective/df itself (hb_gauss_ll_post)"
    if a_frag is None or not skip_a:
        return None, "A is exchanged row-major, or read elsewhere"
    post = plan._gll_post.get(g.id)
    grads = [c for c in plan._consumers.get(node.outputs[1], []) if c.op == "sgp_grad"]
    if len(grads) != 1 or len(plan._consumers.get(node.outputs[1], [])) != 1:
        return None, "A does not feed exactly one sgp_grad"
    gn = grads[0]
    if _through(gn.inputs[8]) is not post[1]:
        return None, "the backward's fbar is not the head's own dobjective/df"
    same = all(gn.inputs[i] is node.inputs[j] for i, j in ((0, 0), (1, 1), (2, 2), (3, 4), (4, 5)))
    if not (same and gn.inputs[5] is node.outputs[3] and gn.inputs[7] is node.outputs[2] and gn.attrs["mode"] == node.attrs["mode"]):
        return None, "the backward does not read this draw's operands, eps and v"
    if not plan.needed(gn.outputs[0]):
        return None, "Lbar is not needed"
    hit, why = _phi_direct_match(plan, gn, a_frag, prec, plan.needed(gn.outputs[4]))
    if hit is None:
        return None, "the backward is not Phi-direct: " + why
    return gn, None


def _phi_direct_match(plan, node, a_frag, prec, need_x):
    H = plan.H
    if a_frag is None:
        return None, "A is exchanged row-major (no column-strip form, or A / xbar is read elsewhere)"
    if plan.dtype != plan.torch.float32 or prec != H.PREC_NATIVE or need_x:
        return None, "needs fp32 operands in native precision"
    Lb, skipped = node.outputs[0], []

    def private(t):
        return len(plan._consumers.get(t, [])) == 1 and t not in plan.outputs and t not in plan._bind

    if not private(Lb):
        return None, "Lbar is a plan output, or has a reader besides the Cholesky VJP's product"
    c = plan._consumers[Lb][0]
    t = Lb
    if c.op == "matutil" and c.attrs["mode"] == MATUTIL_BAND and c.attrs["lower"] < 0 and c.attrs["upper"] == 0:
        t = c.outputs[0]
        if not private(t):
            return None, "tril(Lbar) is a plan output, or has a second reader"
        skipped.append(c.id)
        c = plan._consumers[t][0]
    at = c.attrs
    if not (c.op == "matmul" and len(c.inputs) == 2 and c.inputs[1] is t and c.inputs[0] is not t and at["ta"] and not at["tb"]
            and at["act"] == "none" and not at.get("actgrad")):
        return None, "Lbar does not feed the product L^T tril(Lbar)"
    L, Q = c.inputs[0], c.outputs[0]
    Wsrc, fwd = _through(node.inputs[3], ("stop_gradient",)), node.inputs[6].node
    if not (Wsrc.node.op == "trinv" and Wsrc.node.inputs[0] is L and fwd.op == "sgp" and fwd.inputs[3] is L
            and _through(fwd.inputs[4], ("stop_gradient",)) is Wsrc):
        return None, "the product's left operand is not the factor L whose inverse whitened the draw"
    if not private(Q) or c.id in plan._colsum_of or c.id in plan._mm_head:
        return None, "L^T tril(Lbar) is a plan output, or has a reader besides Phisym"
    mu = plan._consumers[Q][0]
    if not (mu.op == "matutil" and mu.attrs["mode"] == MATUTIL_SYMLOW):
        return None, "L^T tril(Lbar) is not followed by Phisym (matutil mode 4)"
    E, M, n, d, P = _sgp_extents(node)
    if not H.sgp_bwd_phi_supported(E, n, M, d, P):
        return None, "shape outside the column-strip form, or switched off (hb_debug_set sgp_phi_direct 0)"
    return (mu, skipped + [c.id, mu.id]), None


def _sgp_grad_emit(plan, node):
    H = plan.H
    x, z, ell, W, u, eps, A, v, gf = (plan.buf(t) for t in node.inputs)
    mode = SGP_MODES[node.attrs["mode"]]
    if plan.needed(node.outputs[0]):
        a_frag, fprec = plan._afrag.get(node.inputs[6], (None, None))
        hit, why = _phi_direct_match(plan, node, a_frag, fprec, plan.needed(node.outputs[4]))
        plan.note(PHI_DIRECT, node, hit is not None, why or "")
        if hit is not None:
            mu, skipped = hit
            plan._phi_direct.update(skipped)
            wfrag = plan._wfrag[_through(node.inputs[3], ("stop_gradient",))][0]
            outs = (plan.out(mu.outputs[0]),) + tuple(plan.out(t) for t in node.outputs[1:4])
            fused = plan._fwd_kbar.get(node.id)
            if fused is not None:
# ... 444 lines not shown
            for nd in list(c.nodes):
                if nd.op != "strided":
                    continue
                o = nd.outputs[0]
                if o in outputs or any(member.get(x.id) is not c for x in consumers.get(o, [])) or not consumers.get(o):
                    c.nodes.remove(nd)
                    del member[nd.id]
                    changed = True
        ids = {nd.id for nd in c.nodes}
        ext_in = {t for nd in c.nodes for t in nd.inputs if t.node.id not in ids}
        outs = [o for nd in c.nodes for o in nd.outputs if nd.op != "strided"
                and (o in outputs or any(x.id not in ids for x in consumers.get(o, [])))]
        keep = (any(nd.op in ("reduce", "strided") for nd in c.nodes) and sum(1 for nd in c.nodes if nd.op in ("ew", "reduce")) >= 2
                and len(ext_in) <= EW_COL_MAX_IN and 1 <= len(outs) <= EW_COL_MAX_OUT)
        if not keep:
            for nd in c.nodes:
                del member[nd.id]
            c.nodes = []
    return member


INFO_POOL_WORDS = 65536


class CholeskyError(ArithmeticError):
    """A Cholesky factorisation met a non-positive pivot (TensorFlow raises
    InvalidArgumentError from tf.cholesky at the same point)."""


class Plan:

    def __init__(self, outputs, dtype, device, leaf_resolver, rngs, binds=None, prologue=None, stream=None):
        from . import hip_ops
        import torch

        self.H, self.torch = hip_ops, torch
        self.dtype, self.device = dtype, device
        self.outputs = list(outputs)
        self.steps: List = []
        self._buf: Dict[Tensor, object] = {}
        self._bind: Dict[Tensor, object] = {}
        self._rngs = rngs
        self._infos: List[Tuple[object, str]] = []
        self._nocap: List[str] = []
        self._graph = None
        self._graphs: Dict[object, object] = {}
        self._capture_enabled = False
        self._info_pool = None
        self._info_used = 0
        self.stream = stream
        self.side_effect_steps = set()
        self.explain = []
        self.param_only_steps = []
        self.prologue = []
        self.trail_version = None
        self.chain_kind: Dict[int, str] = {}
        self.chain_members: Dict[int, list] = {}
        self._chains_fused = False
        self.step_labels = {}
        self.step_nodes = {}
        self.step_riders: Dict[int, Node] = {}
        self.noise_inputs: Dict[Tensor, object] = {}
        self._injected: Dict[Tensor, bool] = {}
        self._leaf_resolver = leaf_resolver
        self._order = order = topo_order(self.outputs)
        self._order_pos = {n.id: i for i, n in enumerate(order)}
        self._consumers = consumer_map(order)
        self._needed = set(self._consumers) | set(self.outputs)
        self._extra_copies = []
        self._gll_post: Dict[int, tuple] = {}
        self._absorbed = set()
        self._colclusters, self._clusters = {}, {}
        self._sgp_head: Dict[int, Node] = {}
        self._mm_head: Dict[int, Node] = {}
        self._gll_in_sgp: Dict[int, Node] = {}
        self._place: Dict[Tensor, object] = {}
        self._colsum_of: Dict[int, Node] = {}
        self._fused_colsum = set()
        self._fused_trinv, self._fused_matutil, self._fused_concat = set(), set(), set()
        self._wfrag: Dict[Tensor, object] = {}
        self._afrag: Dict[Tensor, object] = {}
        self._phi_direct = set()
        self._fwd_kbar: Dict[int, tuple] = {}
        self._lazy_cols: Dict[Tensor, object] = {}
        self._gll_fused: Dict[int, tuple] = {}
        self._pending: List[tuple] = []
        self._gram_for_chol: Dict[int, tuple] = {}
        self._gram_in_mm: Dict[int, tuple] = {}
        self._gram_tiles: Dict[int, tuple] = {}
        self._chol_rider: Dict[Tensor, dict] = {}
        self._mlp2: Dict[int, dict] = {}
        self._emitted: List[Node] = []
        self._side_cands: List[dict] = []
        for t, b in (binds or []):
            self._prebind(t, b)
        if prologue:
            prologue(self)
        consumers, fuse, jit = self._consumers, _runtime("fuse_elementwise"), hip_ops.ewise_jit_enabled()
        notes = [("elementwise fusion", None, False, "settings.runtime.fuse_elementwise is off")]
        if fuse:
            self._gll_post, self._absorbed, notes = _match_gauss_ll_tails(order, consumers, set(self.outputs))
        self._colclusters = cluster_columns(order, outputs=self.outputs, skip=self._absorbed,
                                            enabled=fuse and jit and _runtime("column_programs"))
        self._clusters = cluster_elementwise(order, enabled=fuse, skip=set(self._colclusters) | self._absorbed,
                                             max_elems=EW_CLUSTER_MAX_ELEMS_JIT if jit else EW_CLUSTER_MAX_ELEMS)
        if fuse and _runtime("head_in_contraction"):
            before = _emitted_before(order, self._clusters, self._colclusters, self.side_jobs_enabled())
            heads, nt = _match_head_in_contraction(order, before)
            self._sgp_head = {sg.id: g for sg, g in heads.items()}
            self._gll_in_sgp = {g.id: sg for sg, g in heads.items()}
            notes += nt
            if _runtime("head_in_decoder"):
                heads, nt = _match_head_in_decoder(order, consumers, self.outputs, self._bind, before, set(self._gll_in_sgp),
                                                   lambda n, k, m: hip_ops.matmul_gauss_units(n, k, m, dtype))
                self._mm_head = {mm.id: g for mm, g in heads.items()}
                self._gll_in_sgp.update((g.id, mm) for mm, g in heads.items())
                notes += nt
        for tgt, (o, off) in _match_concat_placement(order, consumers, self._colclusters, self.outputs, self._bind).items():
            self._place[tgt] = self.out(o).reshape(-1)[off:off + tgt.size].view(tgt.shape)
        self._colsum_of, self._fused_colsum, nt = _match_colsum(order, consumers, self._clusters)
        for entry in notes + nt:
            self.note(*entry)
        self._lower()

    def _lower(self):
        hoist = self.side_jobs_enabled()
        for n in self._order:
            if hoist and n.op == "leaf:minibatch":
                self._emit(n)
        for n in self._order:
            if hoist and n.op == "leaf:minibatch":
                continue
            if n.id in self._absorbed:
                self._emitted.append(n)
                continue
            cc = self._colclusters.get(n.id)
            if cc is not None:
                if n is cc.nodes[-1]:
                    self._flush_pending([t for m in cc.nodes for t in m.inputs])
                    if self._emit_colcluster(cc):
                        self._emitted.extend(cc.nodes)
                continue
            c = self._clusters.get(n.id)
            if c is None or len(c.nodes) < 2:
                self._flush_pending(n.inputs)
                self._emit(n)
            elif n is c.nodes[-1]:
                self._flush_pending([t for m in c.nodes for t in m.inputs])
                self._emit_cluster(c)
                self._emitted.extend(c.nodes)
        self._flush_pending(None)
        for t, b in list(self._bind.items()) + self._extra_copies:
            got = self._buf.get(t)
            if got is not None and got.data_ptr() != b.data_ptr():
                self.steps.append(lambda src=got, b=b: self.H.ewise("COPY", [src.reshape(b.shape)], out=b))

    def _prebind(self, t, b):
        n = t.node
        if n.op == "reshape":
            self._prebind(n.inputs[0], b.view(n.inputs[0].shape))
            return
        b = b.view(t.shape) if tuple(b.shape) != t.shape else b
        if t in self._bind:
            self._extra_copies.append((t, b))
        else:
            self._bind[t] = b
# ... 481 lines not shown
```

henbun_amd/hip_ops.py:

```python
from __future__ import annotations

import collections
import ctypes
from ctypes import c_double, c_int, c_long, c_void_p

import numpy as np
import torch

from . import _lib

_C = _lib.constants()


def _hb(*names):
    return [_C["HB_" + n] for n in names]


EW = {k[len("HB_EW_"):]: v for k, v in _C.items() if k.startswith("HB_EW_") and k != "HB_EW_PROG_SUM"}
RED_SUM, RED_MAX = _hb("RED_SUM", "RED_MAX")
KERN_RBF, KERN_CSYM_RBF, KERN_SQDIST = _hb("KERN_RBF", "KERN_CSYM_RBF", "KERN_SQDIST")
KERN_KBAR_SYMMETRIC = _C["HB_KERN_KBAR_SYMMETRIC"]
EW_PROG_SUM = _C["HB_EW_PROG_SUM"]
COLPROG_SUM, COLPROG_MAX = _hb("COLPROG_SUM", "COLPROG_MAX")
MM_LOWER_OUT, MM_TRIL_OUT, MM_PHI_OUT, MM_SYM_OUT = _hb("MM_LOWER_OUT", "MM_TRIL_OUT", "MM_PHI_OUT", "MM_SYM_OUT")
# ... 243 lines not shown
                pass


def gauss_ll(x, f, scale, var, out=None, post=None, fbar=None):
    _chk(x), _chk(f), _chk(var)
    assert x.numel() == f.numel() and var.numel() == 1 and (scale is None or scale.numel() == 1)
    n = x.numel()
    if out is None:
        ll = _empty(1, dtype=x.dtype, device=x.device)
        dmu = _empty_like(x)
        ds = _empty(1, dtype=x.dtype, device=x.device)
        dv = _empty(1, dtype=x.dtype, device=x.device)
    else:
        ll, dmu, ds, dv = out
    ws = workspace(x.dtype, x.device, 3 * max((n + 1023) // 1024, 1))
    if fbar is not None:
        _chk(fbar)
        assert fbar.numel() == n
        _lib.lib().call("hb_gauss_ll_post" + _suf(x), _p(x), _p(f), _p(scale), _p(var), n, _p(ll), _p(dmu), _p(ds), _p(dv),
                        float(post), _p(fbar), _p(ws), ws.numel(), stream())
        return ll, dmu, ds, dv
    _lib.lib().call("hb_gauss_ll" + _suf(x), _p(x), _p(f), _p(scale), _p(var), n, _p(ll), _p(dmu), _p(ds), _p(dv), _p(ws),
                    ws.numel(), stream())
    return ll, dmu, ds, dv


def reduce_mid(x, K1, R, K2, op=RED_SUM, out=None):
    _chk(x)
    assert x.numel() == K1 * R * K2
    if out is None:
        out = _empty(K1 * K2, dtype=x.dtype, device=x.device)
    ws = workspace(x.dtype, x.device)
    _lib.lib().call("hb_reduce" + _suf(x), op, _p(x), _p(out), K1, R, K2, _p(ws), ws.numel(), stream())
    return out


def copy_nd(src, src_strides, dst, dst_strides, shape, src_off=0, dst_off=0):
    es = src.element_size()
    sp = c_void_p(src.data_ptr() + src_off * es)
    dp = c_void_p(dst.data_ptr() + dst_off * es)
    nd = len(shape)
    _lib.lib().call("hb_copy_nd" + _suf(src), sp, _larr(src_strides) if nd else _larr([0]), dp,
                    _larr(dst_strides) if nd else _larr([0]), nd, _larr(shape) if nd else _larr([1]), stream())
    return dst


def fill(t, value):
    _lib.lib().call("hb_fill" + _suf(t), _p(t), t.numel(), float(value), stream())
    return t


def gather_rows(src, idx, perm=None, out=None, err=None):
    _chk(src)
    nsrc = src.shape[0]
    row = src.numel() // max(nsrc, 1)
    n = idx.numel()
    if out is None:
        out = _empty((n,) + tuple(src.shape[1:]), dtype=src.dtype, device=src.device)
    assert idx.dtype == torch.int64 and (perm is None or perm.dtype == torch.int64)
    _lib.lib().call("hb_gather_rows" + _suf(src), _p(src), nsrc, row, _p(idx), _p(perm), n, _p(out), _p(err), stream())
    return out


class MultiGather:

    def __init__(self, srcs, outs, idx, perm, err):
        assert 1 <= len(srcs) <= 8 and len(srcs) == len(outs)
        nsrc = srcs[0].shape[0]
        for s in srcs:
            _chk(s)
            assert s.shape[0] == nsrc and s.dtype == srcs[0].dtype
        self.suf = _suf(srcs[0])
        self.narr, self.nsrc, self.n = len(srcs), nsrc, idx.numel()
        self.srcs = (c_void_p * self.narr)(*[s.data_ptr() for s in srcs])
        self.dsts = (c_void_p * self.narr)(*[o.data_ptr() for o in outs])
        self.rows = _larr([s.numel() // max(nsrc, 1) for s in srcs])
        self.idx, self.perm, self.err = idx, perm, err
        self._keep = (srcs, outs)

    def launch(self, use_perm=True):
        _lib.lib().call("hb_gather_rows_multi" + self.suf, self.narr, self.srcs, self.rows, self.dsts, self.nsrc,
                        _p(self.idx), _p(self.perm if use_perm else None), self.n, _p(self.err), stream())

    def launch_draw(self, rng, lo, hi, use_perm=True, defer=False):
        name = "hb_side_push_gather_draw_f32" if (defer and self.suf == "_f32") else "hb_gather_rows_multi_draw" + self.suf
        _lib.lib().call(name, self.narr, self.srcs, self.rows, self.dsts, self.nsrc,
                        _p(rng.state), rng.nlanes, int(lo), int(hi), _p(self.idx), _p(self.perm if use_perm else None),
                        self.n, _p(self.err), stream())


def matutil(x, mode, lower=-1, upper=-1, alpha=0.0, out=None):
    _chk(x)
    R, C = x.shape[-2], x.shape[-1]
    B = x.numel() // max(R * C, 1)
    if out is None:
        out = _empty_like(x)
    _lib.lib().call("hb_matutil" + _suf(x), _p(x), _p(out), B, R, C, mode, lower, upper, float(alpha), stream())
    return out


class Rng:

    def __init__(self, seed, stream_id=0, nlanes=65536, device="cuda"):
        self.nlanes = int(nlanes)
        self.state = _empty(2 * self.nlanes, dtype=torch.int64, device=device)
        self.seed, self.stream_id = int(seed), int(stream_id)
        self.reseed(seed, stream_id)

    def reseed(self, seed, stream_id=0):
        self.seed, self.stream_id = int(seed), int(stream_id)
        _lib.lib().call("hb_rng_init", _p(self.state), self.nlanes, int(seed) & (2**64 - 1),
                        int(stream_id) & (2**64 - 1), stream())

    def normal(self, shape, dtype=torch.float32, out=None):
        if out is None:
            out = _empty(shape, dtype=dtype, device=self.state.device)
        _lib.lib().call("hb_rng_normal" + _suf(out), _p(self.state), self.nlanes, _p(out), out.numel(), stream())
        return out

    def randint(self, n, lo, hi, out=None):
        if out is None:
            out = _empty(n, dtype=torch.int64, device=self.state.device)
        _lib.lib().call("hb_rng_randint", _p(self.state), self.nlanes, _p(out), out.numel(), int(lo), int(hi), stream())
        return out


def _rng_args(rng):
    if rng is None:
        return None, 0
    return _p(rng.state), rng.nlanes


def side_flush():
    _lib.lib().call("hb_side_flush", stream())


def side_pending():
    return int(_lib.lib().raw("hb_side_pending")())


def chain_begin():
    _lib.lib().call("hb_chain_begin")


def chain_end():
    _lib.lib().call("hb_chain_end", stream())


def chain_discard():
    return int(_lib.lib().raw("hb_chain_discard")())


def chain_source():
    buf = ctypes.create_string_buffer(1 << 16)
    _lib.lib().call("hb_chain_source", buf, 1 << 16)
    return buf.value.decode()


def side_discard():
    return int(_lib.lib().raw("hb_side_discard")())


def diag_sample_kl_fwd(mu, s, u_in=None, rng=None, out=None, rows=None, defer=False):
    _chk(mu), _chk(s)
    if rows is None:
        n = mu.numel()
        L = ldm = lds = max(n, 1)
# ... 1500 lines not shown
```

henbun_amd/model.py:

```python
from __future__ import annotations

from functools import wraps

import numpy as np

from . import graph as G
from ._settings import settings
from .param import Data, MinibatchData, Parameterized, Variable, graph_key
from . import parallel
from .session import Indexer, Session


class AdamOptimizer:

    def __init__(self, learning_rate=0.001, beta1=0.9, beta2=0.999, epsilon=1e-08, name="Adam"):
        self.learning_rate, self.beta1, self.beta2, self.epsilon = learning_rate, beta1, beta2, epsilon
        self._slots = {}

    def slots(self, session):
        key = (id(session), session.layout_version)
        s = self._slots.get(key)
        if s is None:
            torch = session.torch
            n = session.theta.numel()
# ... 50 lines not shown
            for d in mb:
                if d.data_size != mb[0].data_size:
                    raise ValueError("Minibatch data" + d.long_name + " is not the same size.")
        if len(mb) > 0:
            data_size = mb[0].data_size
            if self._index.data_size is None or self._index.data_size != data_size:
                self._index.setUp(data_size)

    def test_feed_dict(self, minibatch_size=None):
        return self.get_feed_dict(self._index.test_index(minibatch_size))


class AutoOptimize:

    def __call__(self, method):
        @wraps(method)
        def runnable(instance):
            name = "_" + method.__name__ + "_AF_optimizer"
            d = object.__getattribute__(instance, "__dict__")
            if name not in d:
                object.__setattr__(instance, name, Optimizer(instance, method))
            return d[name]

        return runnable


_DEFAULT_ADAM = AdamOptimizer()
STATE_FORMAT_VERSION = 2


class Optimizer:
    def __init__(self, model_instance, likelihood_method):
        self.model = model_instance
        self.likelihood_method = likelihood_method
        self.method_op = None
        self.optimize_op = None
        self._optimizer = None
        self._collection = graph_key.VARIABLES
        self._plans = {}
        self.dp_reduce = "mean"
        self.last_plan = None

    def _trace(self, minibatch):
        sess = self.model._session
        sess.trace_minibatch = minibatch
        try:
            with self.model.tf_mode():
                obj = self.likelihood_method(self.model)
        finally:
            sess.trace_minibatch = None
        if not isinstance(obj, G.Tensor):
            obj = G.constant(np.asarray(obj, dtype=np.float64))
        if obj.size != 1:
            raise ValueError("the objective must be a scalar, got shape %s" % (obj.shape,))
        return G.reshape(obj, [])

    def compile(self, optimizer=_DEFAULT_ADAM, collection=graph_key.VARIABLES, global_step=None, dp_reduce="mean"):
        print("compiling...")
        self._optimizer = optimizer
        self._collection = collection
        self.dp_reduce = dp_reduce
        self._plans = {}
        self.model.initialize()
        mbs = [d for d in self.model.get_variables(graph_key.DATA) if isinstance(d, MinibatchData)]
        probe = None
        if mbs:
            self.model._setup_index()
            probe = min(2, self.model._index.train_size)
        self.model._session.probing = True
        try:
            self.method_op = self._trace(probe)
        finally:
            self.model._session.probing = False
        self.model.validate()
        self.optimize_op = True
        print("finished.")

    def _settings_key(self):
        n = settings.numerics
        return (n.jitter_level, n.clip_by_value, n.clip_value_min, n.clip_value_max, str(getattr(n, "kl_form", "mc")), str(getattr(n, "contraction", "native")),
                str(settings.runtime.index_source), bool(settings.runtime.fuse_elementwise),
                bool(getattr(settings.runtime, "force_dp", False)), str(getattr(settings.runtime, "dp_exchange", "auto")),
                str(getattr(settings.runtime, "ewise", "jit")), bool(getattr(settings.runtime, "side_jobs", True)),
                bool(getattr(settings.runtime, "serial_chains", True)))

    @staticmethod
    def _dp_active(sess):
        return sess.world_size > 1 or bool(getattr(settings.runtime, "force_dp", False))

    def dp_objective(self):
        plan = self.last_plan
        if plan is None or getattr(plan, "dp_mode", "none") == "none":
            return None
        plan.stream.synchronize() if plan.stream is not None else plan.torch.cuda.synchronize()
        sess = self.model._session
        return float(plan.gflat[sess.theta.numel()].item()) / max(sess.world_size, 1)

    def _get_plan(self, kind, minibatch, training=True):
        sess = self.model._session
        self.model.initialize()
        key = (kind, minibatch, training, sess.layout_version, self._settings_key())
        plan = self._plans.get(key)
        if plan is not None:
            return plan
        if minibatch is not None:
            self.model._setup_index()
        obj = self._trace(minibatch)
        if kind == "run":
            plan = sess.make_plan([obj], minibatch=minibatch, training=training)
            plan.objective = obj
        else:
            leaves = []
            for t in self.model.get_tf_variables(self._collection):
                if t is not None and t.node.op == "leaf:param" and t not in leaves:
                    leaves.append(t)
            grads = [g if g is None or not g.node.op.startswith("leaf:") else G.unary("COPY", g)
                     for g in G.gradients(obj, leaves)]
            torch = sess.torch
            P = sess.theta.numel()
            gflat = torch.zeros(P + 2, dtype=sess.torch_dtype, device=sess.device)
            binds, segs = [], []
            for t, g in zip(leaves, grads):
                o, s = sess._offsets[id(t.node.attrs["var"])]
                segs.append((o, s))
                if g is not None:
                    binds.append((g, gflat[o:o + s]))
            outs = [obj] + [g for g in grads if g is not None]
            plan = sess.make_plan(outs, binds=binds, minibatch=minibatch, training=True)
            plan.objective = obj
            plan.gflat = gflat
            segs.sort()
            merged = []
            for o, s in segs:
                if merged and merged[-1][0] + merged[-1][1] == o:
                    merged[-1] = (merged[-1][0], merged[-1][1] + s)
                else:
                    merged.append((o, s))
            plan.segments = merged
            opt = self._optimizer
            slots = opt.slots(sess)
            H = sess.H
            theta = sess.theta
            gscale = -parallel.gradient_scale(sess.world_size, self.dp_reduce)

            info = plan.info_words()
            plan.fail = slots["fail"]

            def adam():
                for i, (o, s) in enumerate(merged):
                    H.adam_step(theta[o:o + s], gflat[o:o + s], slots["m"][o:o + s], slots["v"][o:o + s], slots["t"],
                                lr=opt.learning_rate, b1=opt.beta1, b2=opt.beta2, eps=opt.epsilon, gscale=gscale,
                                tick=(i == len(merged) - 1), info=info, dpflag=plan.dpflag, fail=slots["fail"])

            plan.dpflag = None
            plan.adam = adam
            plan.chain_kind[id(adam)] = "full"
            plan.eager_tail = []
            plan.dp_mode = "none"
            if not self._dp_active(sess):
                plan.steps.append(adam)
                plan.side_effect_steps.add(adam)
            else:
                tail, objbuf = gflat[P:P + 2], plan.buf(obj)
                plan.dpflag = gflat[P + 1:P + 2]

                def pack():
                    H.dp_pack(tail, objbuf, info)
# ... 192 lines not shown
```

henbun_amd/session.py:

```python
from __future__ import annotations

import os
from typing import Dict, List, Optional

import numpy as np

from . import graph as G
from ._settings import np_float_type, settings


class Indexer:

    def __init__(self):
        self.data_size = None
        self.test_frac = 0.1

    def setUp(self, data_size):
        self.data_size = data_size
        self.test_size = int(np.floor(self.data_size * self.test_frac))
        self.train_size = data_size - self.test_size
        index = np.arange(self.data_size)
        np.random.shuffle(index)
        self._train_index = index[: self.train_size]
        self._test_index = index[self.train_size:]
# ... 97 lines not shown
            self.torch.distributed.broadcast(self.theta, 0)
        self._layout = layout
        self._offsets = {id(v): (o, s) for v, o, s in layout}
        self.layout_version += 1
        self.param_version += 1

    def initialize(self):
        self.ensure_layout()
        dirty = False
        for v, o, s in self._layout:
            if v._assigned:
                self.write_raw(v, v._host_raw)
                v.finalize()
                dirty = True
        if dirty and self.world_size > 1:
            self.torch.distributed.broadcast(self.theta, 0)

    def param_view(self, v):
        o, s = self._offsets[id(v)]
        return self.theta[o:o + s].view(tuple(v._full_shape))

    def read_raw(self, v):
        o, s = self._offsets[id(v)]
        self.torch.cuda.synchronize()
        return self.theta[o:o + s].detach().cpu().numpy().astype(np.float64).reshape(v._full_shape)

    def write_raw(self, v, raw):
        o, s = self._offsets[id(v)]
        arr = np.array(np.broadcast_to(np.asarray(raw, dtype=self.np_dtype), v._full_shape))
        self.torch.cuda.synchronize()
        self.theta[o:o + s].copy_(self.torch.as_tensor(arr.reshape(-1)).to(self.device))
        self.torch.cuda.synchronize()
        self.param_version += 1

    def read_value(self, v):
        self.ensure_layout()
        if v._assigned:
            self.write_raw(v, v._host_raw)
            v.finalize()
        return np.asarray(v.transform.forward(self.read_raw(v)))

    def data_buffer(self, var):
        self._ensure_device()
        b = self._data_bufs.get(id(var))
        if b is None:
            arr = np.ascontiguousarray(np.asarray(var.data, dtype=self.np_dtype))
            b = self.torch.as_tensor(arr).to(self.device)
            self._data_bufs[id(var)] = b
        return b

    def data_changed(self, var):
        b = self._data_bufs.get(id(var))
        if b is not None:
            arr = np.ascontiguousarray(np.asarray(var.data, dtype=self.np_dtype))
            b.copy_(self.torch.as_tensor(arr).to(self.device))

    def make_plan(self, outputs, binds=None, minibatch=None, training=True):
        self._ensure_device()
        self.ensure_layout()
        sess = self
        feeder = {"idx": None, "emitted": False}

        def resolver_with_plan(plan):
            def resolve(t):
                kind = t.node.op[5:]
                var = t.node.attrs["var"]
                if kind == "param":
                    if id(var) not in sess._offsets:
                        raise RuntimeError("parameter %s is not part of model %s" % (var.long_name, sess.model.name))
                    return sess.param_view(var)
                if kind == "data":
                    return sess.data_buffer(var)
                if kind == "minibatch":
                    full = sess.data_buffer(var)
                    n = t.shape[0]
                    if minibatch is None:
                        if n != full.shape[0]:
                            raise ValueError("traced with minibatch size %d but run with all %d rows" % (n, full.shape[0]))
                        return full
                    out = sess.torch.empty(t.shape, dtype=sess.torch_dtype, device=sess.device)
                    index = sess.model._index
                    if index.data_size is None or index.data_size != full.shape[0]:
                        sess.model._setup_index()
                    if feeder["idx"] is None:
                        feeder["idx"] = sess.torch.zeros(n, dtype=sess.torch.int64, device=sess.device)
                        feeder["err"] = sess.torch.zeros(1, dtype=sess.torch.int32, device=sess.device)
                        key = "train" if training else "test"
                        perm = index._dev.get(key)
                        if perm is None:
                            src = index._train_index if training else index._test_index
                            perm = sess.torch.as_tensor(np.ascontiguousarray(src, dtype=np.int64)).to(sess.device)
                            index._dev[key] = perm
                        feeder["perm"] = perm
                        hi = index.train_size if training else index.test_size
                        idx, rng = feeder["idx"], sess.rngs["index"]
                        plan.index_buffer = idx
                        plan.index_range = hi
                        if str(settings.runtime.index_source) == "device":
                            feeder["draw"] = (rng, hi)

                            def draw():
                                feeder["drawn"] = False
                                if not plan.indices_injected and not (feeder.get("mg") and n <= rng.nlanes):
                                    rng.randint(n, 0, hi, out=idx)
                                    feeder["drawn"] = True
                            plan.steps.append(draw)
                    idx, perm, err = feeder["idx"], feeder["perm"], feeder["err"]
                    H = sess.H
                    if "arrays" not in feeder:
                        feeder["arrays"] = []
                        feeder["leaves"] = []
                        feeder["cell"] = plan.side_candidate(feeder["leaves"])

                        def gather():
                            mg = feeder.get("mg")
                            if mg is None:
                                srcs = [a for a, _ in feeder["arrays"]]
                                outs = [o for _, o in feeder["arrays"]]
                                if len(srcs) <= 8 and len({tuple(a.shape[:1]) for a in srcs}) == 1:
                                    mg = feeder["mg"] = H.MultiGather(srcs, outs, idx, perm, err)
                                else:
                                    mg = feeder["mg"] = False
                            fused = (mg and feeder.get("draw") and not feeder.get("drawn") and not plan.indices_injected
                                     and n <= feeder["draw"][0].nlanes)
                            if fused:
                                mg.launch_draw(feeder["draw"][0], 0, feeder["draw"][1], use_perm=not plan.indices_raw,
                                               defer=feeder["cell"]["defer"])
                            elif mg:
                                mg.launch(use_perm=not plan.indices_raw)
                            else:
                                for a, o in feeder["arrays"]:
                                    H.gather_rows(a, idx, None if plan.indices_raw else perm, out=o, err=err)

                        plan.steps.append(gather)
                    feeder["arrays"].append((full, out))
                    feeder["leaves"].append(t)
                    plan.gather_err = err
                    return out
                raise RuntimeError("unknown leaf kind " + kind)

            return resolve

        plan = _SessionPlan.__new__(_SessionPlan)
        plan.index_buffer = None
        plan.index_range = None
        plan.indices_injected = False
        plan.indices_raw = False
        plan.gather_err = None
        plan.host_indices = str(settings.runtime.index_source) != "device"
        plan.session = self
        plan.training = training
        self.torch.cuda.synchronize()
        G.Plan.__init__(plan, outputs, self.torch_dtype, self.device, resolver_with_plan(plan), self.rngs, binds=binds,
                        stream=self.stream)
        self.torch.cuda.synchronize()
        return plan


class _SessionPlan(G.Plan):

    def set_indices(self, idx, raw=True):
        if self.index_buffer is None:
            raise ValueError("this plan draws no minibatch")
        idx = np.asarray(idx, dtype=np.int64).reshape(-1)
        if idx.shape[0] != self.index_buffer.shape[0]:
            raise ValueError("expected %d indices, got %d" % (self.index_buffer.shape[0], idx.shape[0]))
        self.torch.cuda.synchronize()
        self.index_buffer.copy_(self.torch.as_tensor(idx).to(self.device))
        self.torch.cuda.synchronize()
        self.indices_injected, self.indices_raw = True, raw
        self._graph = self._graphs.get(self._state_key())

    def clear_indices(self):
        if self.indices_injected:
            self.indices_injected, self.indices_raw = False, False
            self._graph = self._graphs.get(self._state_key())

    def _state_key(self):
        return (G.Plan._state_key(self), self.indices_injected, self.indices_raw)

    def check(self):
        G.Plan.check(self)
        err = getattr(self, "gather_err", None)
        if err is not None and (self.indices_injected or self.host_indices):
            if int(err.cpu().item()) != 0:
                err.zero_()
                raise IndexError("minibatch indices outside the data set (rows were zero-filled)")

    def run(self):
        if self.host_indices and self.index_buffer is not None and not self.indices_injected:
            index = self.session.model._index
            n = self.index_buffer.shape[0]
            pos = np.random.randint(0, self.index_range, n)
            with self._on_stream():
                self.index_buffer.copy_(self.torch.as_tensor(pos).to(self.device), non_blocking=False)
        G.Plan.run(self)
```

include/henbun_hip.h:

```cpp
#ifndef HENBUN_HIP_H
#define HENBUN_HIP_H

#include <stdint.h>

#ifdef __cplusplus
extern "C" {
#endif

#define HB_ABI_VERSION 2

int hb_version(void);
const char* hb_last_error_string(void);
int hb_debug_set(const char* key, long value);
int hb_debug_clear(void);
int hb_device_info(char* buf, int buflen, int* cu_count);

int hb_graph_begin_capture(void* stream);
int hb_graph_end_capture(void* stream, void** exec_out);
int hb_graph_launch(void* exec, void* stream);
int hb_graph_destroy(void* exec);

enum {
  HB_EW_NEG = 1, HB_EW_EXP, HB_EW_LOG, HB_EW_SQRT, HB_EW_SQUARE, HB_EW_ABS, HB_EW_SIGN,
  HB_EW_SIGMOID, HB_EW_RELU, HB_EW_SOFTPLUS, HB_EW_TANH, HB_EW_RECIP, HB_EW_RSQRT,
// ... 413 lines not shown
int hb_gram_predict_grad_f32(int kind, const float* x, const float* x2, const float* ell, long dl, const float* V, long P,
                             double scale, double prior, int acq, double best, double param, int largest, double var_floor,
                             float* mean, float* var, float* val, float* dmean, float* dvar, float* dval, long n, long N,
                             long d, long S, float* ws, void* stream);
int hb_gram_predict_grad_f64(int kind, const double* x, const double* x2, const double* ell, long dl, const double* V, long P,
                             double scale, double prior, int acq, double best, double param, int largest, double var_floor,
                             double* mean, double* var, double* val, double* dmean, double* dvar, double* dval, long n, long N,
                             long d, long S, double* ws, void* stream);
int hb_pcg_dot_f32(const float* a, const float* b, double* out, long S, long N, void* stream);
int hb_pcg_dot_f64(const double* a, const double* b, double* out, long S, long N, void* stream);
int hb_pcg_update_f32(float* x, float* r, const float* p, const float* Ap, const double* rz, double* rr, const double* thr,
                      long S, long N, void* stream);
int hb_pcg_update_f64(double* x, double* r, const double* p, const double* Ap, const double* rz, double* rr, const double* thr,
                      long S, long N, void* stream);
int hb_pcg_direction_f32(const float* r, const float* w, float* p, double* rz, const double* rr, const double* thr,
                         double wscale, double zscale, int first, long S, long N, void* stream);
int hb_pcg_direction_f64(const double* r, const double* w, double* p, double* rz, const double* rr, const double* thr,
                         double wscale, double zscale, int first, long S, long N, void* stream);
int hb_pcg_update_coef_f32(float* x, float* r, const float* p, const float* Ap, const double* rz, double* rr,
                           const double* thr, long S, long N, double* coef, long it, void* stream);
int hb_pcg_update_coef_f64(double* x, double* r, const double* p, const double* Ap, const double* rz, double* rr,
                           const double* thr, long S, long N, double* coef, long it, void* stream);
int hb_pcg_direction_coef_f32(const float* r, const float* w, float* p, double* rz, const double* rr, const double* thr,
                              double wscale, double zscale, int first, long S, long N, double* coef, long it, void* stream);
int hb_pcg_direction_coef_f64(const double* r, const double* w, double* p, double* rz, const double* rr, const double* thr,
                              double wscale, double zscale, int first, long S, long N, double* coef, long it, void* stream);
long hb_gram_bilinear_grad_ws_elems(long N, long dl);
int hb_gram_bilinear_grad_f32(int kind, const float* x, const float* ell, long dl, const float* A, const float* B,
                              const double* w, double* g, long N, long d, long S, double* ws, void* stream);
int hb_gram_bilinear_grad_f64(int kind, const double* x, const double* ell, long dl, const double* A, const double* B,
                              const double* w, double* g, long N, long d, long S, double* ws, void* stream);
long hb_sgp_select_ws_elems(long N, long M, long d, int dtype_bytes);
int hb_sgp_select_f32(int kind, const float* X, const float* ell, long dl, long N, long M, long d, double threshold, long* idx,
                      float* pivots, long* count, double* trace, float* ws, void* stream);
int hb_sgp_select_f64(int kind, const double* X, const double* ell, long dl, long N, long M, long d, double threshold,
                      long* idx, double* pivots, long* count, double* trace, double* ws, void* stream);
long hb_sgp_kgrad_ws_elems(long N, long M, long d, long P);
int hb_sgp_kgrad_f32(int kind, const float* X, const float* Y, const double* z, const double* ell, long dl, const double* Q,
                     const double* R, double* zbar, double* ellbar, long N, long M, long d, long P, double* ws, void* stream);
int hb_sgp_kgrad_f64(int kind, const double* X, const double* Y, const double* z, const double* ell, long dl, const double* Q,
                     const double* R, double* zbar, double* ellbar, long N, long M, long d, long P, double* ws, void* stream);
int hb_sgp_wkgrad_f32(int kind, const float* X, const double* w, const double* r, const double* z, const double* ell, long dl,
                      const double* Q, const double* R, double* zbar, double* ellbar, long N, long M, long d, double* ws,
                      void* stream);
int hb_sgp_wkgrad_f64(int kind, const double* X, const double* w, const double* r, const double* z, const double* ell, long dl,
                      const double* Q, const double* R, double* zbar, double* ellbar, long N, long M, long d, double* ws,
                      void* stream);
int hb_sgp_bwd_f32(int kind, int mode, const float* x, long sx, const float* z, const float* ell,
                   long dl, const float* W, const float* Wfrag, int prec, const float* u, const float* eps,
                   const float* A, const float* A_frag, const float* v, const float* fbar, float* Kbar,
                   float* Kbar_frag, float* Lbar, float* ubar, float* zbar, float* ellbar, float* xbar,
                   long E, long n, long M, long d, long P, float* ws, void* stream);
int hb_sgp_bwd_phi_supported(long E, long n, long M, long d, long P);
int hb_sgp_bwd_phi_f32(int kind, int mode, const float* x, long sx, const float* z, const float* ell, long dl,
                       const float* W, const float* Wfrag, const float* u, const float* eps, const float* A_frag,
                       const float* v, const float* fbar, float* Abar_frag, float* Phi, float* ubar, float* zbar,
                       float* ellbar, long E, long n, long M, long d, long P, float* ws, void* stream);
int hb_sgp_fwd_kbar_supported(long E, long n, long M, long d, long P, int prec, int has_wfrag, int draw, long rng_lanes);
int hb_sgp_fwd_gauss_kbar_f32(int kind, int mode, const float* x, long sx, const float* z, const float* ell, long dl,
                              const float* W, const float* Wfrag, int prec, const float* u, const float* eps_in,
                              uint64_t* rng, long rng_lanes, float* eps_out, float* A, float* A_frag, float* f, float* v,
                              long E, long n, long M, long d, long P, float* ws, const float* y, const float* scale,
                              const float* var, double post, float* dmu, float* fbar, float* head_part, long units,
                              float* Abar_frag, float* bws, void* stream);
int hb_sgp_bwd_phi_rest_f32(const float* A_frag, const float* Abar_frag, float* Phi, float* ubar, float* zbar,
                            float* ellbar, long dl, long E, long n, long M, long d, long P, float* bws, void* stream);
int hb_sgp_bwd_f64(int kind, int mode, const double* x, long sx, const double* z, const double* ell,
                   long dl, const double* W, const double* Wfrag, int prec, const double* u,
                   const double* eps, const double* A, const double* A_frag, const double* v,
                   const double* fbar, double* Kbar, double* Kbar_frag, double* Lbar, double* ubar,
                   double* zbar, double* ellbar, double* xbar, long E, long n, long M, long d, long P,
                   double* ws, void* stream);

int hb_adam_step_f32(float* theta, const float* g, float* m, float* v, long n, double lr, double b1,
                     double b2, double eps, double gscale, long* t, int tick, const int* info,
                     long n_info, const float* dpflag, long* fail, void* stream);
int hb_adam_step_f64(double* theta, const double* g, double* m, double* v, long n, double lr,
                     double b1, double b2, double eps, double gscale, long* t, int tick,
                     const int* info, long n_info, const double* dpflag, long* fail, void* stream);

int hb_side_push_gather_draw_f32(int narr, const float* const* srcs, const long* rows, float* const* dsts, long nsrc,
                                 uint64_t* state, long nlanes, long lo, long hi, long* idx_out, const long* perm,
                                 long n, int* err, void* stream);
int hb_side_push_diag_fwd_f32(const float* mu, const float* s, const float* u_in, uint64_t* rng, long rng_lanes,
                              float* u_out, float* x, float* kl, long n, long L, long ld_mu, long ld_s, float* ws,
                              void* stream);
int hb_side_push_diag_bwd_f32(const float* s, const float* u, const float* x, const float* xbar, const float* klbar,
                              float* mubar, float* sbar, long n, long L, long ld_s, long ld_out, void* stream);
int hb_side_pending(void);
int hb_side_flush(void* stream);
int hb_side_discard(void);

int hb_chain_begin(void);
int hb_chain_end(void* stream);
int hb_chain_discard(void);
int hb_chain_source(char* out, long cap);
int hb_chain_compile_dry(void);
int hb_chain_stamps(unsigned long long* out, long cap);

#define HB_COMM_ID_BYTES 128
int hb_comm_available(void);
int hb_comm_unique_id(char* id128);
int hb_comm_init(const char* id128, int rank, int world, void** comm_out);
int hb_comm_destroy(void* comm);
int hb_allreduce_sum_f32(float* buf, long n, void* comm, void* stream);
int hb_allreduce_sum_f64(double* buf, long n, void* comm, void* stream);
int hb_dp_pack_f32(float* tail, const float* objective, const int* info, long n_info, void* stream);
int hb_dp_pack_f64(double* tail, const double* objective, const int* info, long n_info, void* stream);

#ifdef __cplusplus
}
#endif
#endif
```

Before: 47.12 million samples/s.

## Sort minibatch by key coordinate and skip all-zero kernel chunks in fused SGP strip

Adds a sorted gather-draw side job that orders the drawn minibatch rows by one input coordinate, so that strips of nearby points share locality against the inducing points. The fused forward/Kbar strip kernel now records which 32-wide inducing chunks have any nonzero kernel value and skips the MMA work for chunks that are entirely zero, writing zeros directly for those retirements. The sort path is off by default (sort_minibatch defaults to False), while chunk skipping is on by default and costs a ballot/atomicOr plus mask bookkeeping. Without sorting, random 1-D points in an 8192-point batch rarely leave whole chunks zero, so the skip may seldom fire.

```diff
diff --git a/henbun_amd/csrc/elementwise.hip b/henbun_amd/csrc/elementwise.hip
--- a/henbun_amd/csrc/elementwise.hip
+++ b/henbun_amd/csrc/elementwise.hip
@@ -724,6 +724,47 @@
   return gather_rows_multi_draw<float>(narr, srcs, rows, dsts, nsrc, state, nlanes, lo, hi, idx_out, perm, n, err,
                                        (hipStream_t)stream, true);
 }
+extern "C" long hb_gather_sorted_max(void) { return HB_SORT_MAX; }
+static int gather_rows_multi_draw_sorted(int narr, const float* const* srcs, const long* rows, float* const* dsts, long nsrc,
+                                         int key, uint64_t* state, long nlanes, long lo, long hi, long* idx_out,
+                                         const long* perm, long n, int* err, hipStream_t stream, bool defer) {
+  HB_REQUIRE(narr >= 1 && narr <= HB_GATHER_MAX, "hb_gather_rows_multi_draw_sorted: %d arrays (max %d)", narr, HB_GATHER_MAX);
+  HB_REQUIRE(n >= 0 && nsrc >= 0 && srcs && rows && dsts && state && idx_out, "hb_gather_rows_multi_draw_sorted: bad arguments");
+  HB_REQUIRE(key >= 0 && key < narr, "hb_gather_rows_multi_draw_sorted: key array %d of %d", key, narr);
+  HB_REQUIRE(n <= nlanes, "hb_gather_rows_multi_draw_sorted: n=%ld exceeds the %ld RNG lanes", n, nlanes);
+  HB_REQUIRE(n <= HB_SORT_MAX, "hb_gather_rows_multi_draw_sorted: n=%ld exceeds %d (hb_gather_sorted_max)", n, HB_SORT_MAX);
+  HB_REQUIRE(hi > lo, "hb_gather_rows_multi_draw_sorted: empty range [%ld,%ld)", lo, hi);
+  HbSideJob j;
+  memset(&j, 0, sizeof(j));
+  j.kind = HB_SIDE_GATHER_SORTED, j.nblocks = 1;
+  j.gather.g.narr = narr;
+  for (int a = 0; a < HB_GATHER_MAX; ++a) {
+    const int from = a == 0 ? key : (a == key ? 0 : a);
+    j.gather.g.src[a] = a < narr ? srcs[from] : nullptr;
+    j.gather.g.dst[a] = a < narr ? dsts[from] : nullptr;
+    j.gather.g.row[a] = a < narr ? rows[from] : 1;
+    if (a < narr) HB_REQUIRE(rows[from] >= 1 && srcs[from] && dsts[from], "hb_gather_rows_multi_draw_sorted: bad array %d", from);
+  }
+  if (n == 0) return 0;
+  j.gather.state = state, j.gather.nlanes = nlanes, j.gather.lo = lo, j.gather.range = (uint64_t)(hi - lo);
+  j.gather.idx_out = idx_out, j.gather.perm = perm, j.gather.n = n, j.gather.nsrc = nsrc, j.gather.err = err;
+  j.gather.G = 1, j.gather.key = key;
+  const int rc = hb_side_push(j, stream);
+  if (rc || defer) return rc;
+  return hb_side_flush((void*)stream);
+}
+extern "C" int hb_gather_rows_multi_draw_sorted_f32(int narr, const float* const* srcs, const long* rows, float* const* dsts,
+                                                    long nsrc, int key, uint64_t* state, long nlanes, long lo, long hi,
+                                                    long* idx_out, const long* perm, long n, int* err, void* stream) {
+  return gather_rows_multi_draw_sorted(narr, srcs, rows, dsts, nsrc, key, state, nlanes, lo, hi, idx_out, perm, n, err,
+                                       (hipStream_t)stream, false);
+}
+extern "C" int hb_side_push_gather_draw_sorted_f32(int narr, const float* const* srcs, const long* rows, float* const* dsts,
+                                                   long nsrc, int key, uint64_t* state, long nlanes, long lo, long hi,
+                                                   long* idx_out, const long* perm, long n, int* err, void* stream) {
+  return gather_rows_multi_draw_sorted(narr, srcs, rows, dsts, nsrc, key, state, nlanes, lo, hi, idx_out, perm, n, err,
+                                       (hipStream_t)stream, true);
+}
 extern "C" int hb_gather_rows_multi_draw_f64(int narr, const double* const* srcs, const long* rows, double* const* dsts,
                                              long nsrc, uint64_t* state, long nlanes, long lo, long hi, long* idx_out,
                                              const long* perm, long n, int* err, void* stream) {
diff --git a/henbun_amd/csrc/linalg.hip b/henbun_amd/csrc/linalg.hip
--- a/henbun_amd/csrc/linalg.hip
+++ b/henbun_amd/csrc/linalg.hip
@@ -577,7 +577,9 @@
   const bool sym = (a.flags & HB_MM_SYM_OUT) != 0;
   const long nt = a.M / 32;
   const int nown = (int)(sym ? nt * (nt + 1) / 2 : (a.M / 32) * (a.N / 32));
-  const HbSideJobs sj = hb_side_take();
+  int src = 0;
+  const HbSideJobs sj = hb_side_take(stream, false, &src);
+  if (src) return src;
   dim3 grid((unsigned)(nown + sj.total), (unsigned)a.batch, 1);
 #define HB_WGK(TA_, TB_)                                                                                   \
   do {                                                                                                     \
@@ -2166,11 +2168,12 @@
   float diag = 0.f;
 };
 __global__ void __launch_bounds__(512, 2) chol_persist_kernel(CpArgs a, HbSideJobs side) {
+  __shared__ __attribute__((aligned(16))) char lds[sizeof(CpLds) > HB_SORT_LDS_BYTES ? sizeof(CpLds) : HB_SORT_LDS_BYTES];
   if ((int)blockIdx.x >= a.total) {
+    if (hb_side_run_sorted(side, (int)blockIdx.x - a.total, lds, 512)) return;
     if (threadIdx.x < 256) hb_side_run(side, (int)blockIdx.x - a.total);
     return;
   }
-  __shared__ __attribute__((aligned(16))) char lds[sizeof(CpLds)];
   __shared__ unsigned s_ticket;
   if (threadIdx.x == 0) s_ticket = __hip_atomic_fetch_add(&a.sync[0], 1u, __ATOMIC_RELAXED, __HIP_MEMORY_SCOPE_AGENT);
   __syncthreads();
@@ -2196,7 +2199,9 @@
 #else
   a.stamps = nullptr;
 #endif
-  const HbSideJobs sj = hb_side_take();
+  int src = 0;
+  const HbSideJobs sj = hb_side_take(stream, hb_sgp_rider_pending() == 0, &src);
+  if (src) return src;
   const int rr = hb_sgp_rider_launch_with(a, sj, stream);
   if (rr != 0) return rr < 0 ? rr : 0;
   hipLaunchKernelGGL(chol_persist_kernel, dim3((unsigned)(a.total + sj.total)), dim3(512), 0, stream, a, sj);
@@ -2257,7 +2262,9 @@
     HbSideJobs noside = {};
     for (int k = 0; k < nrt / 2; ++k) {
       const int nown = chol64_grid(nrt, k, inv);
-      const HbSideJobs sj = k == 0 ? hb_side_take() : noside;
+      int src = 0;
+      const HbSideJobs sj = k == 0 ? hb_side_take(stream, false, &src) : noside;
+      if (src) return src;
       dim3 grid((unsigned)(nown + (k == 0 ? sj.total : 0)), (unsigned)B);
       hipLaunchKernelGGL(chol_rl64_kernel, grid, dim3(256), 0, stream, (const float*)A, (float*)L,
                          inv ? (float*)ws : (float*)nullptr, (float*)W, (int)M, k, info, nown, sj);
diff --git a/henbun_amd/csrc/runtime.hip b/henbun_amd/csrc/runtime.hip
--- a/henbun_amd/csrc/runtime.hip
+++ b/henbun_amd/csrc/runtime.hip
@@ -94,23 +94,49 @@
 
 __global__ void __launch_bounds__(256) hb_side_jobs_kernel(HbSideJobs J) { hb_side_run(J, (int)blockIdx.x); }
 
+__global__ void __launch_bounds__(256) hb_side_jobs_sorted_kernel(HbSideJobs J) {
+  __shared__ __attribute__((aligned(16))) char lds[HB_SORT_LDS_BYTES];
+  if (hb_side_run_sorted(J, (int)blockIdx.x, lds, 256)) return;
+  hb_side_run(J, (int)blockIdx.x);
+}
+
+static bool hb_side_has_sorted(const HbSideJobs& J) {
+  for (int q = 0; q < J.n; ++q)
+    if (J.job[q].kind == HB_SIDE_GATHER_SORTED) return true;
+  return false;
+}
+
 static int hb_side_launch(const HbSideJobs& J, hipStream_t stream) {
   if (J.n == 0 || J.total == 0) return 0;
-  hipLaunchKernelGGL(hb_side_jobs_kernel, dim3((unsigned)J.total), dim3(256), 0, stream, J);
+  if (hb_side_has_sorted(J))
+    hipLaunchKernelGGL(hb_side_jobs_sorted_kernel, dim3((unsigned)J.total), dim3(256), 0, stream, J);
+  else
+    hipLaunchKernelGGL(hb_side_jobs_kernel, dim3((unsigned)J.total), dim3(256), 0, stream, J);
   HB_LAUNCH_CHECK();
   return 0;
 }
 
-HbSideJobs hb_side_take() {
+static HbSideJobs hb_side_take_all() {
   HbSideJobs J = hb_side_list;
   hb_side_list.n = 0;
   hb_side_list.total = 0;
   return J;
 }
 
+HbSideJobs hb_side_take(hipStream_t stream, bool sorted_ok, int* rc) {
+  HbSideJobs J = hb_side_take_all();
+  if (rc) *rc = 0;
+  if (!sorted_ok && hb_side_has_sorted(J)) {
+    const int r = hb_side_launch(J, stream);
+    if (rc) *rc = r;
+    J.n = 0, J.total = 0;
+  }
+  return J;
+}
+
 int hb_side_push(const HbSideJob& job, hipStream_t stream) {
   if (hb_side_list.n == HB_SIDE_MAX) {
-    const HbSideJobs J = hb_side_take();
+    const HbSideJobs J = hb_side_take_all();
     const int rc = hb_side_launch(J, stream);
     if (rc) return rc;
   }
@@ -127,6 +153,6 @@
   return n;
 }
 extern "C" int hb_side_flush(void* stream) {
-  const HbSideJobs J = hb_side_take();
+  const HbSideJobs J = hb_side_take_all();
   return hb_side_launch(J, (hipStream_t)stream);
 }
diff --git a/henbun_amd/csrc/sgp.hip b/henbun_amd/csrc/sgp.hip
--- a/henbun_amd/csrc/sgp.hip
+++ b/henbun_amd/csrc/sgp.hip
@@ -1252,6 +1252,7 @@
   bool bwd_strip;
   bool bwd_phi;
   bool fwd_kbar;
+  bool skip_zero;
   SgpWs ws;
 };
 static SgpForm sgp_form(int call, int elem_bytes, long E, long n, long M, long d, long P, int prec, bool has_wfrag, bool w_aligned,
@@ -1265,6 +1266,7 @@
   const bool early = hb_debug_get("sgp_early", 1) != 0;
   const bool phi_direct = hb_debug_get("sgp_phi_direct", 1) != 0;
   const bool fwd_kbar = hb_debug_get("sgp_fwd_kbar", 1) != 0;
+  const bool skip_zero = hb_debug_get("sgp_skip_zero", 1) != 0;
   SgpForm f;
   f.ws = sgp_ws(E, n, M, d, P);
   const bool fp32 = elem_bytes == 4, bf16x3 = prec == HB_PREC_BF16X3;
@@ -1288,6 +1290,7 @@
   f.bwd_strip = fp32 && has_wfrag && !want_xbar && f.path && f.ws.strip_elems <= f.ws.mm_elems;
   f.bwd_phi = !bf16x3 && f.path && phi_direct;
   f.fwd_kbar = f.head_units > 0 && f.bwd_phi && f.bwd_strip && d <= SGP_FK_DMAX && E * nS <= SGP_FK_MAX_STRIPS && fwd_kbar;
+  f.skip_zero = skip_zero;
   return f;
 }
 static inline SgpForm sgp_form_query(long E, long n, long M, long d, long P, int prec, bool has_wfrag, bool draw, long rng_lanes) {
@@ -1306,6 +1309,7 @@
   const float* WTf;
   float* part;
   float* Abf;
+  int skip_zero;
 };
 static int sgp_fwd_kbar_launch(SgpArgs<float> a, SgpFwdKbar k, long E, hipStream_t stream);
 
@@ -1725,7 +1729,9 @@
           HB_REQUIRE(form.fwd_kbar && a.head && a.hfbar && A_frag, "hb_sgp_fwd_gauss_kbar: not served here (hb_sgp_fwd_kbar_supported), or fbar / A_frag missing");
           HB_REQUIRE(!A, "hb_sgp_fwd_gauss_kbar: A is exchanged fragment-major only (pass A = NULL)");
           HB_REQUIRE(!g_rider.armed, "hb_sgp_fwd_gauss_kbar after hb_sgp_rider_begin: the fused call does not ride");
-          return sgp_fwd_kbar_launch(a, *fk, E, stream);
+          SgpFwdKbar kk = *fk;
+          kk.skip_zero = form.skip_zero ? 1 : 0;
+          return sgp_fwd_kbar_launch(a, kk, E, stream);
         }
         if (g_rider.armed) {
           HB_REQUIRE(form.record, "hb_sgp_fwd after hb_sgp_rider_begin: this call cannot ride (hb_sgp_rider_supported)");
@@ -2377,6 +2383,7 @@
   __shared__ __attribute__((aligned(16))) float cjs[SGP_SN];
   __shared__ __attribute__((aligned(16))) float fbs[1][SGP_SN];
   __shared__ float lred[(SGP_STRIP_THREADS / 64) * D];
+  __shared__ unsigned s_live;
   float (*Ks)[SGP_SLD] = reinterpret_cast<float (*)[SGP_SLD]>(lds_raw);
   long e;
   int bx;
@@ -2392,7 +2399,6 @@
   const int t1 = nT - 1 - w, t0 = w;
   const int d0 = w < t1 ? w + 1 : 0;
   const int d1 = w <= t1 ? t1 + 1 : 0;
-  const int nts = d0 + d1;
   const bool means = true;
   HB_FSTAMP(0);
   float u0 = 0.f, u1 = 0.f;
@@ -2410,10 +2416,17 @@
 #pragma unroll
     for (int dd = 0; dd < D; ++dd) xss[tid * D + dd] = col.xs[dd];
   }
+  if (tid == 0) s_live = 0u;
   __syncthreads();
-  sgp_strip_fill<D, SGP_STRIP_THREADS>(Ks, zs, col, M, tid);
+  sgp_strip_fill<D, SGP_STRIP_THREADS, true>(Ks, zs, col, M, tid, &s_live);
   __syncthreads();
   HB_FSTAMP(1);
+  const unsigned all_chunks = nT >= 32 ? ~0u : (1u << nT) - 1u;
+  const unsigned live = k.skip_zero ? (unsigned)__builtin_amdgcn_readfirstlane((int)s_live) : all_chunks;
+  const unsigned fm0 = d0 ? live & ((2u << t0) - 1u) : 0u;
+  const unsigned fm1 = d1 ? live & ((2u << t1) - 1u) : 0u;
+  const int n0 = __builtin_popcount(fm0);
+  const int nts = n0 + __builtin_popcount(fm1);
 
   float csq[16], cu[16];
 #pragma unroll
@@ -2444,16 +2457,31 @@
 #pragma unroll
       for (int r = 0; r < 16; ++r) acc[r] = 0.f;
     };
-    auto load = [&](V4 (&f)[4], int ts) {
-      const int tc = ts < nts ? ts : nts - 1;
-      const int tile = tc < d0 ? t0 : t1, Q = tc < d0 ? tc : tc - d0;
+    unsigned lm0 = fm0, lm1 = fm1, cm0 = fm0, cm1 = fm1;
+    int nq = 0;
+    auto settle_zero = [&]() {
+#pragma unroll
+      for (int r = 0; r < 16; ++r) acc[r] += 0.f;
+    };
+    auto load = [&](V4 (&f)[4]) {
+      if (!(lm0 | lm1)) return;
+      const bool first = lm0 != 0u;
+      const int tile = first ? t0 : t1;
+      const unsigned m = first ? lm0 : lm1, rest = m & (m - 1u);
+      const int Q = __builtin_ctz(m);
+      lm0 = first ? rest : 0u, lm1 = first ? lm1 : rest;
       const float* p = Wf + ((long)(tile * nT + Q) << 10) + 4 * lane;
 #pragma unroll
       for (int v = 0; v < 4; ++v) f[v] = *reinterpret_cast<const V4*>(p + 256 * v);
     };
     auto compute = [&](const V4 (&f)[4], int ts) {
       if (ts >= nts) return;
-      const int Q = ts < d0 ? ts : ts - d0;
+      const bool first = cm0 != 0u;
+      const unsigned m = first ? cm0 : cm1, rest = m & (m - 1u);
+      const int Q = __builtin_ctz(m);
+      cm0 = first ? rest : 0u, cm1 = first ? cm1 : rest;
+      if (Q != nq) settle_zero();
+      nq = Q + 1;
       V4 bv[4];
 #pragma unroll
       for (int v = 0; v < 4; ++v) bv[v] = *reinterpret_cast<const V4*>(&Ks[li][32 * Q + 16 * h + 4 * v]);
@@ -2461,30 +2489,38 @@
       for (int v = 0; v < 4; ++v)
 #pragma unroll
         for (int s = 0; s < 4; ++s) acc = MM::mma(bv[v][s], f[v][s], acc);
-      if (ts == d0 - 1) retire_fwd(t0, u0, keep0);
+      if (ts == n0 - 1) {
+        if (nq != t0 + 1) settle_zero();
+        retire_fwd(t0, u0, keep0);
+        nq = 0;
+      }
     };
-    if (nts > 0) {
+    if (d1) {
       V4 fa[4], fb[4];
-      load(fa, 0);
+      load(fa);
 #pragma nounroll
       for (int ts = 0; ts < nts; ts += 2) {
-        load(fb, ts + 1);
+        load(fb);
         __builtin_amdgcn_sched_barrier(0);
         compute(fa, ts);
         __builtin_amdgcn_sched_barrier(0);
-        load(fa, ts + 2);
+        load(fa);
         __builtin_amdgcn_sched_barrier(0);
         compute(fb, ts + 1);
         __builtin_amdgcn_sched_barrier(0);
       }
+      if (nq != t1 + 1) settle_zero();
       retire_fwd(t1, u1, keep1);
+      if (d0 && n0 == 0) retire_fwd(t0, u0, keep0);
     }
   }
   HB_FSTAMP(2);
 
   const int ta = nT - 1 - w, tb = w;
-  const int kd0 = ta > tb ? w + 1 : 0;
-  const int kd1 = tb <= ta ? nT - w : 0;
+  const bool own_a = ta > tb, own_b = tb <= ta;
+  const bool live_a = own_a && ((live >> ta) & 1u), live_b = own_b && ((live >> tb) & 1u);
+  const int kd0 = live_a ? w + 1 : 0;
+  const int kd1 = live_b ? nT - w : 0;
   const int knts = kd0 + kd1;
   auto tile_of = [&](int ts) { return ts < kd0 ? ta : tb; };
   auto chunk_of = [&](int ts) { return ts < kd0 ? ta + ts : tb + (ts - kd0); };
@@ -2583,6 +2619,15 @@
       for (int s2 = 0; s2 < 4; ++s2) acc = MM::mma(bv[v][s2], f[v][s2], acc);
     if (ts == kd0 - 1 || ts == knts - 1) retire(tile_of(ts));
   };
+  auto retire_clear = [&](int tile) {
+    if (h == 0) {
+#pragma unroll
+      for (int dd = 0; dd < D; ++dd)
+        part[(long)dd * M + 32 * tile + li] = 0.f * col.sc[dd] * float(1.0 / (SGP_EXP2_SCALE * SGP_EXP2_SCALE));
+    }
+  };
+  if (own_a && !live_a) retire_clear(ta);
+  if (own_b && !live_b) retire_clear(tb);
   if (knts > 0) {
 #pragma nounroll
     for (int ts = 0; ts < knts; ts += 2) {
diff --git a/henbun_amd/csrc/sgp_strip.cuh b/henbun_amd/csrc/sgp_strip.cuh
--- a/henbun_amd/csrc/sgp_strip.cuh
+++ b/henbun_amd/csrc/sgp_strip.cuh
@@ -72,10 +72,12 @@
   }
 };
 
-template <int D, int NTH>
-__device__ __forceinline__ void sgp_strip_fill(float (*Ks)[SGP_SLD], const float* zs, const SgpStripColumn<D>& col, int M, int tid) {
+template <int D, int NTH, bool LIVE = false>
+__device__ __forceinline__ void sgp_strip_fill(float (*Ks)[SGP_SLD], const float* zs, const SgpStripColumn<D>& col, int M, int tid,
+                                               unsigned* live = nullptr) {
   typedef float V4 __attribute__((ext_vector_type(4)));
   const int c = tid & 31, kq = tid >> 5;
+  unsigned mine = 0u;
 #pragma unroll 4
   for (int k4 = kq * 4; k4 < M; k4 += NTH / 8) {
     float zq[4 * D];
@@ -89,6 +91,17 @@
 #pragma unroll
     for (int q = 0; q < 4; ++q) v[q] = col.value(&zq[q * D]);
     *reinterpret_cast<V4*>(&Ks[c][k4]) = v;
+    if constexpr (LIVE) {
+      const unsigned bits = __float_as_uint(v[0]) | __float_as_uint(v[1]) | __float_as_uint(v[2]) | __float_as_uint(v[3]);
+      if (bits != 0u) mine |= 1u << (k4 >> 5);
+    }
+  }
+  if constexpr (LIVE) {
+    unsigned any = 0u;
+#pragma unroll
+    for (int Q = 0; Q < SGP_SM_MAX / 32; ++Q)
+      if (__ballot((mine >> Q) & 1u) != 0ull) any |= 1u << Q;
+    if (any != 0u && (tid & 63) == 0) atomicOr(live, any);
   }
 }
 
diff --git a/henbun_amd/csrc/side_jobs.cuh b/henbun_amd/csrc/side_jobs.cuh
--- a/henbun_amd/csrc/side_jobs.cuh
+++ b/henbun_amd/csrc/side_jobs.cuh
@@ -138,7 +138,7 @@
 }
 
 #define HB_SIDE_MAX 3
-enum { HB_SIDE_GATHER_DRAW = 1, HB_SIDE_DIAG_FWD = 2, HB_SIDE_DIAG_BWD = 3 };
+enum { HB_SIDE_GATHER_DRAW = 1, HB_SIDE_DIAG_FWD = 2, HB_SIDE_DIAG_BWD = 3, HB_SIDE_GATHER_SORTED = 4 };
 struct HbSideGather {
   GatherMultiArgs<float> g;
   uint64_t* state;
@@ -149,7 +149,140 @@
   long n, nsrc;
   int* err;
   int G;
-};
+  int key;
+};
+
+#define HB_SORT_MAX 8192
+#define HB_SORT_LDS_BYTES (HB_SORT_MAX * 8)
+__device__ __forceinline__ unsigned hb_sort_key_image(float key) {
+  if (key != key) return 0xfffffffeu;
+  const unsigned b = __float_as_uint(key + 0.0f);
+  return (b & 0x80000000u) ? ~b : (b | 0x80000000u);
+}
+#define HB_SORT_BATCH 8
+__device__ __forceinline__ void hb_sort_cex(unsigned long long& x0, unsigned long long& x1, bool asc) {
+  const bool sw = (x0 > x1) == asc;
+  const unsigned long long lo = sw ? x1 : x0, hi = sw ? x0 : x1;
+  x0 = lo, x1 = hi;
+}
+__device__ __forceinline__ void gather_sorted_body(const HbSideGather& a, unsigned long long* __restrict__ sl, int nth) {
+  constexpr int NB = HB_SORT_BATCH;
+  const int tid = threadIdx.x, n = (int)a.n;
+  int np = 1;
+  while (np < n) np <<= 1;
+  const float* __restrict__ ksrc = a.g.src[0];
+  const long kw = a.g.row[0];
+  bool anybad = false;
+  for (int base = tid; base < np; base += nth * NB) {
+    HbRng rg[NB];
+    long j[NB], jj[NB];
+    float key[NB];
+#pragma unroll
+    for (int b = 0; b < NB; ++b)
+      if (base + b * nth < n) rg[b] = rng_load(a.state, a.nlanes, base + b * nth);
+#pragma unroll
+    for (int b = 0; b < NB; ++b) {
+      const int r = base + b * nth;
+      if (r < n) {
+        j[b] = a.lo + (long)__umul64hi(rg[b].next(), a.range);
+        rng_store(a.state, a.nlanes, r, rg[b]);
+        a.idx_out[r] = j[b];
+      }
+    }
+#pragma unroll
+    for (int b = 0; b < NB; ++b)
+      if (base + b * nth < n) jj[b] = a.perm ? a.perm[j[b]] : j[b];
+#pragma unroll
+    for (int b = 0; b < NB; ++b) {
+      key[b] = 0.f;
+      if (base + b * nth < n) {
+        const bool bad = jj[b] < 0 || jj[b] >= a.nsrc;
+        anybad = anybad || bad;
+        if (!bad) key[b] = ksrc[jj[b] * kw];
+      }
+    }
+#pragma unroll
+    for (int b = 0; b < NB; ++b) {
+      const int r = base + b * nth;
+      if (r < np) sl[r] = r < n ? (((unsigned long long)hb_sort_key_image(key[b]) << 32) | (unsigned)r) : ~0ull;
+    }
+  }
+  if (anybad && a.err) *a.err = 1;
+  __syncthreads();
+  for (unsigned kk = 2; kk <= (unsigned)np; kk <<= 1) {
+    unsigned jx = kk >> 1;
+    for (; jx >= 2; jx >>= 2) {
+      const unsigned h = jx >> 1;
+      for (unsigned g = tid; g < (unsigned)np / 4; g += nth) {
+        const unsigned i0 = ((g & ~(h - 1)) << 2) | (g & (h - 1));
+        const bool asc = (i0 & kk) == 0;
+        unsigned long long x0 = sl[i0], x1 = sl[i0 | h], x2 = sl[i0 | jx], x3 = sl[i0 | jx | h];
+        hb_sort_cex(x0, x2, asc), hb_sort_cex(x1, x3, asc);
+        hb_sort_cex(x0, x1, asc), hb_sort_cex(x2, x3, asc);
+        sl[i0] = x0, sl[i0 | h] = x1, sl[i0 | jx] = x2, sl[i0 | jx | h] = x3;
+      }
+      __syncthreads();
+    }
+    if (jx == 1) {
+      for (unsigned i = tid; i < (unsigned)np / 2; i += nth) {
+        const unsigned lo = i << 1;
+        unsigned long long x0 = sl[lo], x1 = sl[lo | 1];
+        hb_sort_cex(x0, x1, (lo & kk) == 0);
+        sl[lo] = x0, sl[lo | 1] = x1;
+      }
+      __syncthreads();
+    }
+  }
+  for (int base = tid; base < n; base += nth * NB) {
+    unsigned pos[NB];
+    long jv[NB];
+#pragma unroll
+    for (int b = 0; b < NB; ++b)
+      if (base + b * nth < n) pos[b] = (unsigned)sl[base + b * nth];
+#pragma unroll
+    for (int b = 0; b < NB; ++b)
+      if (base + b * nth < n) jv[b] = a.idx_out[pos[b]];
+#pragma unroll
+    for (int b = 0; b < NB; ++b)
+      if (base + b * nth < n) sl[base + b * nth] = (unsigned long long)jv[b];
+  }
+  __syncthreads();
+  for (int base = tid; base < n; base += nth * NB) {
+    long jj[NB];
+    bool bad[NB];
+#pragma unroll
+    for (int b = 0; b < NB; ++b) {
+      const int k = base + b * nth;
+      jj[b] = 0;
+      if (k < n) {
+        jj[b] = (long)sl[k];
+        a.idx_out[k] = jj[b];
+      }
+    }
+    if (a.perm) {
+#pragma unroll
+      for (int b = 0; b < NB; ++b)
+        if (base + b * nth < n) jj[b] = a.perm[jj[b]];
+    }
+#pragma unroll
+    for (int b = 0; b < NB; ++b) bad[b] = jj[b] < 0 || jj[b] >= a.nsrc;
+#pragma unroll
+    for (int q = 0; q < HB_GATHER_MAX; ++q) {
+      if (q >= a.g.narr) break;
+      const long w = a.g.row[q];
+      const float* __restrict__ src = a.g.src[q];
+      float* __restrict__ dst = a.g.dst[q];
+      for (long c = 0; c < w; ++c) {
+        float v[NB];
+#pragma unroll
+        for (int b = 0; b < NB; ++b) v[b] = (base + b * nth < n && !bad[b]) ? src[jj[b] * w + c] : 0.f;
+#pragma unroll
+        for (int b = 0; b < NB; ++b)
+          if (base + b * nth < n) dst[(long)(base + b * nth) * w + c] = v[b];
+      }
+    }
+  }
+}
 struct HbSideDiagFwd {
   const float *mu, *s, *u_in;
   uint64_t* rng;
@@ -198,7 +331,25 @@
   }
 }
 
+__device__ __forceinline__ bool hb_side_run_sorted(const HbSideJobs& J, int vb, void* lds, int nth) {
+  int q = -1, v = vb;
+#pragma unroll
+  for (int i = 0; i < HB_SIDE_MAX; ++i) {
+    const bool open = q < 0 && v >= 0 && i < J.n;
+    if (open && v < J.job[i].nblocks) q = i;
+    if (open) v -= J.job[i].nblocks;
+  }
+  const int kind = q == 0 ? J.job[0].kind : q == 1 ? J.job[1].kind : q == 2 ? J.job[2].kind : 0;
+  static_assert(HB_SIDE_MAX == 3, "the selection below names every slot");
+  if (kind != HB_SIDE_GATHER_SORTED) return false;
+  HbSideGather a = J.job[0].gather;
+  if (q == 1) a = J.job[1].gather;
+  if (q == 2) a = J.job[2].gather;
+  gather_sorted_body(a, reinterpret_cast<unsigned long long*>(lds), nth);
+  return true;
+}
+
 int hb_side_push(const HbSideJob& job, hipStream_t stream);
-HbSideJobs hb_side_take();
+HbSideJobs hb_side_take(hipStream_t stream, bool sorted_ok, int* rc = nullptr);
 
 #endif
diff --git a/henbun_amd/graph.py b/henbun_amd/graph.py
--- a/henbun_amd/graph.py
+++ b/henbun_amd/graph.py
@@ -1810,6 +1810,8 @@
         gn, why = None, "d > 2, more than 512 strips, or switched off (hb_debug_set sgp_fwd_kbar 0)"
     if g is not None:
         plan.note(FWD_KBAR, node, gn is not None, why or "")
+    if g is not None:
+        _sort_minibatch_match(plan, node, gn is not None, d)
     if gn is not None:
         abar_frag = plan.scratch((a_frag.numel(),))
         bws = plan.scratch((H.sgp_ws_elems(E, n, M, d, P),))
@@ -1864,6 +1866,29 @@
 
 PHI_DIRECT = "Cholesky VJP's first product folded into the sparse-GP backward (hb_sgp_bwd_phi)"
 FWD_KBAR = "forward and Kbar column strips in one launch (hb_sgp_fwd_gauss_kbar)"
+
+
+SORT_MINIBATCH = "minibatch rows drawn in order of x (hb_gather_rows_multi_draw_sorted)"
+
+
+def _sort_minibatch_match(plan, node, fused, d):
+    src = _through(node.inputs[0], ("reshape", "stop_gradient"))
+    why = None
+    if not getattr(plan, "sort_minibatch", False):
+        why = "settings.runtime.sort_minibatch is off (or the plan draws no minibatch of a session)"
+    elif not fused:
+        why = "the node does not take the fused forward + Kbar form (FWD_KBAR), the only kernel that skips zero chunks"
+    elif src.node.op != "leaf:minibatch":
+        why = "x is not a minibatch array"
+    elif d != 1:
+        why = "x has %d columns: the rows are ordered by one coordinate only" % d
+    elif getattr(plan, "host_indices", True) or not plan.side_jobs_enabled():
+        why = "the indices are not drawn on the device inside the gather's side job"
+    elif plan.sort_leaf is not None:
+        why = "the draw is already ordered for another node"
+    if why is None:
+        plan.sort_leaf = src
+    plan.note(SORT_MINIBATCH, node, why is None, why or "")
 
 
 def _fwd_kbar_match(plan, node, g, head, a_frag, skip_a, prec):
@@ -2474,6 +2499,7 @@
         self._afrag: Dict[Tensor, object] = {}
         self._phi_direct = set()
         self._fwd_kbar: Dict[int, tuple] = {}
+        self.sort_leaf = None
         self._lazy_cols: Dict[Tensor, object] = {}
         self._gll_fused: Dict[int, tuple] = {}
         self._pending: List[tuple] = []
diff --git a/henbun_amd/hip_ops.py b/henbun_amd/hip_ops.py
--- a/henbun_amd/hip_ops.py
+++ b/henbun_amd/hip_ops.py
@@ -349,7 +349,21 @@
         _lib.lib().call("hb_gather_rows_multi" + self.suf, self.narr, self.srcs, self.rows, self.dsts, self.nsrc,
                         _p(self.idx), _p(self.perm if use_perm else None), self.n, _p(self.err), stream())
 
-    def launch_draw(self, rng, lo, hi, use_perm=True, defer=False):
+    def sorted_supported(self, rng):
+        return self.suf == "_f32" and self.n <= rng.nlanes and self.n <= int(_lib.lib().raw("hb_gather_sorted_max")())
+
+    def launch_draw(self, rng, lo, hi, use_perm=True, defer=False, sort_key=None):
+        if sort_key is not None:
+            perm = _p(self.perm if use_perm else None)
+            if defer:
+                _lib.lib().call("hb_side_push_gather_draw_sorted_f32", self.narr, self.srcs, self.rows, self.dsts, self.nsrc,
+                                int(sort_key), _p(rng.state), rng.nlanes, int(lo), int(hi), _p(self.idx), perm, self.n,
+                                _p(self.err), stream())
+            else:
+                _lib.lib().call("hb_gather_rows_multi_draw_sorted_f32", self.narr, self.srcs, self.rows, self.dsts, self.nsrc,
+                                int(sort_key), _p(rng.state), rng.nlanes, int(lo), int(hi), _p(self.idx), perm, self.n,
+                                _p(self.err), stream())
+            return
         name = "hb_side_push_gather_draw_f32" if (defer and self.suf == "_f32") else "hb_gather_rows_multi_draw" + self.suf
         _lib.lib().call(name, self.narr, self.srcs, self.rows, self.dsts, self.nsrc,
                         _p(rng.state), rng.nlanes, int(lo), int(hi), _p(self.idx), _p(self.perm if use_perm else None),
diff --git a/henbun_amd/model.py b/henbun_amd/model.py
--- a/henbun_amd/model.py
+++ b/henbun_amd/model.py
@@ -156,7 +156,7 @@
                 str(settings.runtime.index_source), bool(settings.runtime.fuse_elementwise),
                 bool(getattr(settings.runtime, "force_dp", False)), str(getattr(settings.runtime, "dp_exchange", "auto")),
                 str(getattr(settings.runtime, "ewise", "jit")), bool(getattr(settings.runtime, "side_jobs", True)),
-                bool(getattr(settings.runtime, "serial_chains", True)))
+                bool(getattr(settings.runtime, "serial_chains", True)), bool(getattr(settings.runtime, "sort_minibatch", False)))
 
     @staticmethod
     def _dp_active(sess):
diff --git a/henbun_amd/session.py b/henbun_amd/session.py
--- a/henbun_amd/session.py
+++ b/henbun_amd/session.py
@@ -203,6 +203,17 @@
                     index = sess.model._index
                     if index.data_size is None or index.data_size != full.shape[0]:
                         sess.model._setup_index()
+                    def ensure_mg():
+                        mg = feeder.get("mg")
+                        if mg is None:
+                            srcs = [a for a, _ in feeder["arrays"]]
+                            outs = [o for _, o in feeder["arrays"]]
+                            if len(srcs) <= 8 and len({tuple(a.shape[:1]) for a in srcs}) == 1:
+                                mg = feeder["mg"] = sess.H.MultiGather(srcs, outs, feeder["idx"], feeder["perm"], feeder["err"])
+                            else:
+                                mg = feeder["mg"] = False
+                        return mg
+
                     if feeder["idx"] is None:
                         feeder["idx"] = sess.torch.zeros(n, dtype=sess.torch.int64, device=sess.device)
                         feeder["err"] = sess.torch.zeros(1, dtype=sess.torch.int32, device=sess.device)
@@ -222,6 +233,8 @@
 
                             def draw():
                                 feeder["drawn"] = False
+                                if getattr(plan, "sort_leaf", None) is not None:
+                                    ensure_mg()
                                 if not plan.indices_injected and not (feeder.get("mg") and n <= rng.nlanes):
                                     rng.randint(n, 0, hi, out=idx)
                                     feeder["drawn"] = True
@@ -234,19 +247,17 @@
                         feeder["cell"] = plan.side_candidate(feeder["leaves"])
 
                         def gather():
-                            mg = feeder.get("mg")
-                            if mg is None:
-                                srcs = [a for a, _ in feeder["arrays"]]
-                                outs = [o for _, o in feeder["arrays"]]
-                                if len(srcs) <= 8 and len({tuple(a.shape[:1]) for a in srcs}) == 1:
-                                    mg = feeder["mg"] = H.MultiGather(srcs, outs, idx, perm, err)
-                                else:
-                                    mg = feeder["mg"] = False
+                            mg = ensure_mg()
                             fused = (mg and feeder.get("draw") and not feeder.get("drawn") and not plan.indices_injected
                                      and n <= feeder["draw"][0].nlanes)
                             if fused:
+                                key = None
+                                leaf = getattr(plan, "sort_leaf", None)
+                                if leaf is not None and mg.sorted_supported(feeder["draw"][0]):
+                                    at = [i for i, t in enumerate(feeder["leaves"]) if t is leaf]
+                                    key = at[0] if at else None
                                 mg.launch_draw(feeder["draw"][0], 0, feeder["draw"][1], use_perm=not plan.indices_raw,
-                                               defer=feeder["cell"]["defer"])
+                                               defer=feeder["cell"]["defer"], sort_key=key)
                             elif mg:
                                 mg.launch(use_perm=not plan.indices_raw)
                             else:
@@ -269,6 +280,7 @@
         plan.indices_raw = False
         plan.gather_err = None
         plan.host_indices = str(settings.runtime.index_source) != "device"
+        plan.sort_minibatch = bool(getattr(settings.runtime, "sort_minibatch", False))
         plan.session = self
         plan.training = training
         self.torch.cuda.synchronize()
diff --git a/include/henbun_hip.h b/include/henbun_hip.h
--- a/include/henbun_hip.h
+++ b/include/henbun_hip.h
@@ -519,6 +519,13 @@
 int hb_side_push_gather_draw_f32(int narr, const float* const* srcs, const long* rows, float* const* dsts, long nsrc,
                                  uint64_t* state, long nlanes, long lo, long hi, long* idx_out, const long* perm,
                                  long n, int* err, void* stream);
+long hb_gather_sorted_max(void);
+int hb_gather_rows_multi_draw_sorted_f32(int narr, const float* const* srcs, const long* rows, float* const* dsts,
+                                         long nsrc, int key, uint64_t* state, long nlanes, long lo, long hi,
+                                         long* idx_out, const long* perm, long n, int* err, void* stream);
+int hb_side_push_gather_draw_sorted_f32(int narr, const float* const* srcs, const long* rows, float* const* dsts,
+                                        long nsrc, int key, uint64_t* state, long nlanes, long lo, long hi,
+                                        long* idx_out, const long* perm, long n, int* err, void* stream);
 int hb_side_push_diag_fwd_f32(const float* mu, const float* s, const float* u_in, uint64_t* rng, long rng_lanes,
                               float* u_out, float* x, float* kl, long n, long L, long ld_mu, long ld_s, float* ws,
                               void* stream);
```

Result: slower. 46.18 million samples/s (-2.0%).
